# vgteam/vg

Measured on AMD Instinct MI355X. Metric: reads/sec aligned (150 bp), higher is better.
Workload: dtype u16

## Files before the change

include/vgk_engine.h:

```cpp
#ifndef VGK_ENGINE_H
#define VGK_ENGINE_H
#include "vgk.h"
#ifdef __cplusplus
extern "C" {
#endif

typedef struct vgk_find_seeds_policy {
    uint32_t hit_cap, hard_hit_cap;  double minimizer_score_fraction;
    uint32_t max_unique_min, num_bp_per_min, minimizer_coverage_flank, exclude_overlapping_min;
    uint32_t minimizer_downsampling_window_count, reserved;  uint64_t minimizer_downsampling_max_window_length;
} vgk_find_seeds_policy;

#define VGK_SEED_TAKEN        0
#define VGK_SEED_DOWNSAMPLED  1
#define VGK_SEED_NO_HITS      2
#define VGK_SEED_HARD_HIT_CAP 3
#define VGK_SEED_OVERLAPPING  4
#define VGK_SEED_MAX_MIN      5
#define VGK_SEED_HIT_CAP      6

int vgk_minimizer_choose(vgk_ctx* ctx, const vgk_find_seeds_policy* policy, uint32_t k, const char* reads, const uint64_t* read_off, uint32_t n,
                         const uint64_t* minimizer_off, const vgk_read_minimizer* minimizers, uint8_t* verdict);

int vgk_minimizer_find_seeds(vgk_ctx* ctx, const vgk_minimizer_index* index, const vgk_find_seeds_policy* policy, const char* reads, const uint64_t* read_off, uint32_t n,
                             uint64_t* minimizer_off, vgk_read_minimizer* minimizers, uint8_t* take, size_t cap_m,
                             uint64_t* seed_off, vgk_seed* seeds, size_t cap_s, size_t written[2]);

double vgk_minimizer_choose_last_ms(vgk_ctx* ctx);

int vgk_batch_refill_stats(vgk_batch* batch, uint64_t out[5]);

#ifdef __cplusplus
}
#endif
#endif
```

vg_amd/capi.py:

```python
import ctypes
import os
import weakref

import numpy as np

_HERE = os.path.dirname(os.path.abspath(__file__))
DEFAULT_LIB = os.path.join(_HERE, "libvgamd.so")

VGK_OK = 0
VGK_EINVAL, VGK_ENODEV, VGK_ENOMEM, VGK_ETOOLONG, VGK_EOVERFLOW, VGK_EOPS = -1, -2, -3, -4, -5, -6
VGK_GSSW_LOCAL = 0
VGK_GSSW_PINNED = 1
VGK_XDROP_PINNED = 2
VGK_GSSW_TRACEBACK = 16
OP_M, OP_I, OP_D, OP_S = 0, 1, 2, 3
OP_CHARS = "MIDS"

GRAPH_DT = np.dtype([("n_nodes", "<u4"), ("_pad", "<u4"), ("node_len", "<u8"), ("seq", "<u8"),
                     ("pred_off", "<u8"), ("pred_idx", "<u8")])
PROBLEM_DT = np.dtype([("read", "<u8"), ("read_len", "<u4"), ("flags", "<u4"), ("graph", GRAPH_DT), ("pinning", "<u8"),
                       ("max_gap_length", "<u4"), ("reserved", "<u4"), ("qual", "<u8")])
RESULT_DT = np.dtype([("score", "<i4"), ("status", "<i4"), ("end_node", "<i4"), ("end_offset", "<i4"),
                      ("end_read", "<i4"), ("first_offset", "<i4"), ("n_ops", "<u4"), ("ops_begin", "<u4")])
OP_DT = np.dtype([("node", "<u4"), ("len", "<u2"), ("op", "u1"), ("pad", "u1")])
# ... 823 lines not shown
        self.read_off = np.asarray(read_off, dtype=np.int64)
        self.seeds = np.ascontiguousarray(seeds, dtype=SEED_DT)
        self.seed_off = np.asarray(seed_off, dtype=np.int64)
        n = self.n = len(self.read_off) - 1
        arr = np.zeros(n, dtype=GAPLESS_DT)
        arr["read"] = self.reads.ctypes.data + self.read_off[:-1]
        arr["read_len"] = np.diff(self.read_off)
        arr["n_seeds"] = np.diff(self.seed_off)
        arr["seeds"] = self.seeds.ctypes.data + 8 * self.seed_off[:-1]
        arr["max_mismatches"] = max_mismatches
        arr["flags"] = np.where(np.broadcast_to(np.asarray(trim), (n,)), VGK_GAPLESS_TRIM, 0)
        arr["overlap_threshold"] = overlap_threshold
        self.array = arr
        rl = np.diff(self.read_off); ns = np.diff(self.seed_off)
        self.ext_cap = int(ns.sum()) + 1
        self.node_cap = int(node_cap if node_cap is not None else (ns * (rl + 2)).sum()) + 1
        self.mism_cap = int(mism_cap if mism_cap is not None else (ns * rl).sum()) + 1

    @classmethod
    def from_lists(cls, problems):
        reads = [np.frombuffer(p["read"].encode(), dtype=np.uint8) for p in problems]
        read_off = np.concatenate([[0], np.cumsum([len(r) for r in reads])]).astype(np.int64)
        read_buf = np.concatenate(reads) if len(reads) and read_off[-1] else np.zeros(1, np.uint8)
        seed_off = np.concatenate([[0], np.cumsum([len(p["seeds"]) for p in problems])]).astype(np.int64)
        seeds = np.zeros(max(int(seed_off[-1]), 1), dtype=SEED_DT)
        k = 0
        for p in problems:
            for node, diff in p["seeds"]:
                seeds[k] = (node, diff); k += 1
        return cls(read_buf, read_off, seeds, seed_off, [p.get("max_mismatches", 4) for p in problems],
                   [p.get("overlap_threshold", 0.8) for p in problems], [p.get("trim", True) for p in problems])


class WfaSet:

    def __init__(self, seqs, seq_off, mode, from_node, from_offset, to_node, to_offset, path_cap=None, edit_cap=None):
        self.seqs = np.ascontiguousarray(seqs, dtype=np.uint8)
        self.seq_off = np.asarray(seq_off, dtype=np.int64)
        n = self.n = len(self.seq_off) - 1
        arr = np.zeros(n, dtype=WFA_DT)
        arr["seq"] = self.seqs.ctypes.data + self.seq_off[:-1]
        arr["seq_len"] = np.diff(self.seq_off)
        arr["mode"] = mode
        arr["from_node"] = from_node; arr["from_offset"] = from_offset
        arr["to_node"] = to_node; arr["to_offset"] = to_offset
        self.array = arr
        sl = np.diff(self.seq_off)
        self.path_cap = int(path_cap if path_cap is not None else (4 * sl + 64).sum()) + 1
        self.edit_cap = int(edit_cap if edit_cap is not None else (2 * sl + 8).sum()) + 1

    @classmethod
    def from_lists(cls, problems):
        modes = {"connect": WFA_CONNECT, "suffix": WFA_SUFFIX, "prefix": WFA_PREFIX}
        seqs = [np.frombuffer(p["seq"].encode(), dtype=np.uint8) for p in problems]
        seq_off = np.concatenate([[0], np.cumsum([len(r) for r in seqs])]).astype(np.int64)
        buf = np.concatenate(seqs) if len(seqs) and seq_off[-1] else np.zeros(1, np.uint8)
        none = (WFA_NO_NODE, 0)
        return cls(buf, seq_off, [modes[p.get("mode", "connect")] for p in problems],
                   [(p.get("from") or none)[0] for p in problems], [(p.get("from") or none)[1] for p in problems],
                   [(p.get("to") or none)[0] for p in problems], [(p.get("to") or none)[1] for p in problems])


class HaploIndex:

    def __init__(self, eng, nodes, threads=None, gbwt=None):
        self.eng = eng
        if isinstance(nodes, tuple):
            self.nodes = None
            self._len = np.ascontiguousarray(nodes[0], dtype=np.uint32); self._seq = np.ascontiguousarray(nodes[1], dtype=np.uint8)
            nodes = self._len
        else:
            self.nodes = list(nodes)
            self._len = np.array([len(s) for s in nodes], dtype=np.uint32)
            self._seq = np.frombuffer("".join(nodes).encode(), dtype=np.uint8).copy()
        if gbwt is not None:
            h = ctypes.c_void_p()
            eng.lib.vgk_haplo_create_gbwt.argtypes = [ctypes.c_void_p, ctypes.c_char_p, ctypes.c_size_t, ctypes.c_uint32, ctypes.c_void_p, ctypes.c_void_p, ctypes.c_void_p]
            eng._check(eng.lib.vgk_haplo_create_gbwt(eng.h, bytes(gbwt), len(gbwt), len(nodes), self._len.ctypes.data, self._seq.ctypes.data, ctypes.byref(h)),
                       "vgk_haplo_create_gbwt")
            self.h = h
            eng._indexes.add(self)
            return
        self._toff = np.concatenate([[0], np.cumsum([len(t) for t in threads])]).astype(np.uint32)
        self._tn = np.ascontiguousarray(np.concatenate([np.asarray(t, dtype=np.uint32) for t in threads]) if len(threads) and self._toff[-1] else np.zeros(1, np.uint32), dtype=np.uint32)
        d = Haplotypes(len(nodes), self._len.ctypes.data, self._seq.ctypes.data, len(threads), self._toff.ctypes.data, self._tn.ctypes.data)
        h = ctypes.c_void_p()
        eng._check(eng.lib.vgk_haplo_create(eng.h, ctypes.byref(d), ctypes.byref(h)), "vgk_haplo_create")
        self.h = h
        eng._indexes.add(self)

    def run_nodes(self):
        self.eng.lib.vgk_haplo_run_nodes.restype = ctypes.c_uint64; self.eng.lib.vgk_haplo_run_nodes.argtypes = [ctypes.c_void_p]
        return int(self.eng.lib.vgk_haplo_run_nodes(self.h))

    def search_nodes(self):
        self.eng.lib.vgk_haplo_search_nodes.restype = ctypes.c_uint64; self.eng.lib.vgk_haplo_search_nodes.argtypes = [ctypes.c_void_p]
        return int(self.eng.lib.vgk_haplo_search_nodes(self.h))

    def close(self):
        if getattr(self, "h", None):
            if getattr(self.eng, "h", None):
                self.eng.lib.vgk_haplo_destroy(self.h)
            self.h = None

    __del__ = close


class Batch:
    def __init__(self, eng, h, ps, ops_per_problem):
        self.eng, self.h, self.ps, self.ops_per = eng, h, ps, ops_per_problem

    def __enter__(self):
        return self

    def __exit__(self, *a):
        self.free()

    def free(self):
        if self.h:
            self.eng.lib.vgk_batch_free(self.h); self.h = None

    def run(self):
        self.eng._check(self.eng.lib.vgk_gssw_run(self.h), "vgk_gssw_run")

    def sync(self):
        self.eng._check(self.eng.lib.vgk_batch_sync(self.h), "vgk_batch_sync")

    def kernel_ms(self, which=-1):
        return self.eng.lib.vgk_batch_kernel_ms(self.h, which)

    def cells(self):
        return self.eng.lib.vgk_batch_cells(self.h)

    def alg_bytes(self):
        return self.eng.lib.vgk_batch_alg_bytes(self.h)

    def device_bytes(self):
        return self.eng.lib.vgk_batch_device_bytes(self.h)

    def lane(self):
        self.eng.lib.vgk_batch_lane.argtypes = [ctypes.c_void_p]
        return self.eng.lib.vgk_batch_lane(self.h)

    def wave_steps(self):
        return self.eng.lib.vgk_batch_wave_steps(self.h)

    def refill_stats(self):
        f = self.eng.lib.vgk_batch_refill_stats
        f.restype = ctypes.c_int; f.argtypes = [ctypes.c_void_p, ctypes.c_void_p]
        out = (ctypes.c_uint64 * 5)()
        self.eng._check(f(self.h, out), "vgk_batch_refill_stats")
        return dict(zip(("waves", "steps", "missed", "bounded", "broken"), (int(v) for v in out)))

    def speculated(self):
        self.eng.lib.vgk_batch_speculated.argtypes = [ctypes.c_void_p]
        return bool(self.eng.lib.vgk_batch_speculated(self.h))

    def fetch(self, into=None):
        n = self.ps.n
        if self.ops_per:
            cap = n * self.ops_per
        else:
            cap = int(np.diff(self.ps.read_off).sum() + np.diff(self.ps.seq_off).sum() + 2 * n)
        if into is not None:
            res, ops = into[0], (into[1].base if into[1].base is not None else into[1])
            assert len(res) == n and len(ops) >= max(cap, 1)
        else:
            res = np.zeros(n, dtype=RESULT_DT)
            ops = np.zeros(max(cap, 1), dtype=OP_DT)
        written = ctypes.c_size_t()
        self.eng._check(self.eng.lib.vgk_gssw_fetch(self.h, res.ctypes.data, ops.ctypes.data, cap, ctypes.byref(written)),
                        "vgk_gssw_fetch")
        return res, ops[:written.value]


def cigar_string(res_row, ops):
    o = ops[res_row["ops_begin"]:res_row["ops_begin"] + res_row["n_ops"]]
    parts, cur = [], None
    for e in o:
        if cur != e["node"]:
            parts.append("%d:" % e["node"]); cur = e["node"]
        parts[-1] += "%d%s" % (e["len"], OP_CHARS[e["op"]])
    return "%d@%s" % (res_row["first_offset"], ",".join(parts))
```

vg_amd/csrc/backend_hip.hip:

```cpp
#include <chrono>
#include <thread>
#include <hip/hip_runtime.h>
#include <cstdlib>
#include <string>
#include "backend.hpp"
#include "pack_hip.hpp"

namespace vgk {

static __device__ __forceinline__ uint32_t from_lane_above(uint32_t x) {
    return (uint32_t)__builtin_amdgcn_update_dpp(0, (int)x, 0x138 , 0xf, 0xf, true);
}

template <int K>
struct TbStage {
    static constexpr uint32_t REC = (K + 3) / 4, RB = REC - 4;
    static constexpr uint32_t DWORDS = TB_TILE * 64u * REC;
    uint32_t* lds;
    __device__ __forceinline__ uint32_t* slot_a(uint32_t t, uint32_t lane) const { const uint32_t s = t % TB_TILE; return lds + (s * 64u + (lane ^ s)) * 4u; }
    __device__ __forceinline__ uint32_t* slot_b(uint32_t t, uint32_t lane) const { return lds + TB_TILE * 64u * 4u + ((t % TB_TILE) * 64u + lane) * RB; }
    __device__ __forceinline__ void flush(uint32_t* tile, uint32_t lane) const {
        __builtin_amdgcn_fence(__ATOMIC_ACQ_REL, "wavefront");
        __builtin_amdgcn_wave_barrier();
#pragma unroll
        for (uint32_t j = 0; j < TB_TILE; ++j) {
            const uint32_t g = j * 64u + lane, L = g / TB_TILE, s = g % TB_TILE;
            const uint4 v = *reinterpret_cast<const uint4*>(lds + (s * 64u + (L ^ s)) * 4u);
            reinterpret_cast<uint4*>(tile)[g] = v;
        }
        if constexpr (RB > 0) {
            uint32_t* part_b = tile + TB_TILE * 64u * 4u;
            const uint32_t* lb = lds + TB_TILE * 64u * 4u;
#pragma unroll
            for (uint32_t j = 0; j < 2u * RB; ++j) {
                const uint32_t q = j * 64u + lane;
                uint4 v; uint32_t* w = reinterpret_cast<uint32_t*>(&v);
#pragma unroll
                for (uint32_t c = 0; c < 4u; ++c) { const uint32_t d = 4u * q + c, r = d / RB, L = r / TB_TILE, st = r % TB_TILE; w[c] = lb[(st * 64u + L) * RB + d % RB]; }
                reinterpret_cast<uint4*>(part_b)[q] = v;
            }
        }
        __builtin_amdgcn_fence(__ATOMIC_ACQ_REL, "wavefront");
        __builtin_amdgcn_wave_barrier();
    }
};

template <int K, bool S8, bool REWALK, bool CODES = true, bool KEY3 = false, bool NOKEY = false>
__global__ __launch_bounds__(256, (K <= 16 ? 4 : 3)) void gssw_fill_kernel(const GsswParams P) {
    constexpr uint32_t REC = (K + 3) / 4;
    __shared__ __attribute__((aligned(16))) uint32_t stage_lds[4][REWALK ? 64u * TB_BND_CHUNK * 2u : (TB_TILE > 1 ? TbStage<K>::DWORDS : 256u)];
    const uint32_t wave = P.wave_begin + blockIdx.x * 4u + (threadIdx.x >> 6);
    const uint32_t lane = threadIdx.x & 63u;
    if (wave >= P.wave_begin + P.wave_count) return;
    if (P.wave_limit && wave - P.wave_begin >= *P.wave_limit) return;
    const WaveDesc wd = P.waves[wave];
    Lane<K> s;
#if VGK_PB_LDS
    __shared__ uint32_t pb_lds[4][64 * K];
    s.PBL = (typename Lane<K>::lds_u32*)(pb_lds[threadIdx.x >> 6] + lane);
#endif
    lane_init<K, NOKEY ? 1 : 0>(s, P, wd, lane);
    asm volatile("" : "+v"(s.one));
    uint32_t* tb = P.want_tb ? P.tb : nullptr;
    TbStage<K> stage{stage_lds[threadIdx.x >> 6]};
    uint32_t steady_from = 0, steady_to = 0;
    if constexpr (!CODES) {
        uint32_t shortest = s.RA < s.RB ? s.RA : s.RB;
#pragma unroll
        for (int d = 32; d > 0; d >>= 1) { const uint32_t o = (uint32_t)__shfl_xor((int)shortest, d, 64); shortest = o < shortest ? o : shortest; }
        steady_steps(wd.G, shortest, wd.n_steps, steady_from, steady_to);
        steady_from = (uint32_t)__builtin_amdgcn_readfirstlane((int)steady_from); steady_to = (uint32_t)__builtin_amdgcn_readfirstlane((int)steady_to);
    }
    if constexpr (!CODES) {
        uint32_t t = 0;
        for (; t < steady_from; ++t) {
            if ((t & 3u) == 0) lane_prefetch(s, P, t);
            const uint32_t rh = from_lane_above(s.out_h), rf = from_lane_above(s.out_f), ri = from_lane_above(s.info);
            lane_step<K, S8, false, KEY3>(s, P, t, rh, rf, ri, nullptr, nullptr);
        }
        for (; t < steady_to; ++t) {
            if ((t & 3u) == 0) lane_prefetch(s, P, t);
            const uint32_t rh = from_lane_above(s.out_h), rf = from_lane_above(s.out_f), ri = from_lane_above(s.info);
            lane_step<K, S8, false, KEY3, false, true>(s, P, t, rh, rf, ri, nullptr, nullptr);
        }
        for (; t < wd.n_steps; ++t) {
            if ((t & 3u) == 0) lane_prefetch(s, P, t);
            const uint32_t rh = from_lane_above(s.out_h), rf = from_lane_above(s.out_f), ri = from_lane_above(s.info);
            lane_step<K, S8, false, KEY3>(s, P, t, rh, rf, ri, nullptr, nullptr);
        }
    }
    for (uint32_t t = 0; CODES && t < wd.n_steps; ++t) {
        if ((t & 3u) == 0) lane_prefetch(s, P, t);
        const uint32_t rh = from_lane_above(s.out_h);
        const uint32_t rf = from_lane_above(s.out_f);
        const uint32_t ri = from_lane_above(s.info);
        if constexpr (!CODES) {
        } else if constexpr (REWALK) {
            lane_step<K, S8, false>(s, P, t, rh, rf, ri, nullptr, nullptr);
            if (tb) {
                uint32_t* st = stage_lds[threadIdx.x >> 6] + lane * (TB_BND_CHUNK * 2u);
                const uint32_t slot = (t ^ lane) & (TB_BND_CHUNK - 1u);
                *reinterpret_cast<uint2*>(st + slot * 2u) = make_uint2(s.out_h, s.out_f);
                if ((t & (TB_BND_CHUNK - 1u)) == TB_BND_CHUNK - 1u || t + 1u == wd.n_steps) {
                    __builtin_amdgcn_fence(__ATOMIC_ACQ_REL, "wavefront"); __builtin_amdgcn_wave_barrier();
                    uint4* out = reinterpret_cast<uint4*>(tb + tb_bnd(wd.tb_off, wd.n_steps, t & ~(TB_BND_CHUNK - 1u), lane));
#pragma unroll
                    for (uint32_t j = 0; j < TB_BND_CHUNK; j += 2) {
                        const uint2 a = *reinterpret_cast<const uint2*>(st + ((j ^ lane) & (TB_BND_CHUNK - 1u)) * 2u), b = *reinterpret_cast<const uint2*>(st + (((j + 1u) ^ lane) & (TB_BND_CHUNK - 1u)) * 2u);
                        out[j >> 1] = make_uint4(a.x, a.y, b.x, b.y);
                    }
                    __builtin_amdgcn_fence(__ATOMIC_ACQ_REL, "wavefront"); __builtin_amdgcn_wave_barrier();
                }
                lane_store_checkpoint<K>(s, P, wd, t, lane);
            }
        } else if constexpr (TB_TILE > 1) {
            lane_step<K, S8, true, false, NOKEY>(s, P, t, rh, rf, ri, tb ? stage.slot_a(t, lane) : nullptr, stage.slot_b(t, lane));
            if (tb && ((t % TB_TILE) == TB_TILE - 1u || t + 1u == wd.n_steps)) stage.flush(tb + tb_tile_base(wd.tb_off, t, REC), lane);
        } else
            lane_step<K, S8, true, false, NOKEY>(s, P, t, rh, rf, ri, tb ? tb + tb_dword(wd.tb_off, t, lane, REC, 0) : nullptr, tb ? tb + tb_dword(wd.tb_off, t, lane, REC, 4) : nullptr);
    }
    if constexpr (NOKEY) return;
    if (REWALK || !CODES || !P.fused) {
#pragma unroll
        for (int half = 0; half < 2; ++half) {
            uint32_t prob; unsigned long long key;
            if (lane_best(s, half, prob, key)) atomicMax(&P.best[prob], key);
        }
        return;
    }
    unsigned long long* mine = reinterpret_cast<unsigned long long*>(stage_lds[threadIdx.x >> 6]);
#pragma unroll
    for (int half = 0; half < 2; ++half) {
        uint32_t prob; unsigned long long key = 0;
        if (!lane_best(s, half, prob, key)) key = 0;
        mine[lane * 2 + half] = key;
    }
    __threadfence();
    const uint32_t n_slots = 2u * (64u / wd.G);
    for (uint32_t slot = lane; slot < n_slots; slot += 64u) {
        const uint32_t q = slot >> 1, half = slot & 1u;
        if (wd.first_pair + q >= wd.pair_end) continue;
        const uint32_t prob = P.order[2u * (wd.first_pair + q) + half];
        if (prob == 0xffffffffu) continue;
        unsigned long long key = 0;
        for (uint32_t g = 0; g < wd.G; ++g) { const unsigned long long k = mine[(q * wd.G + g) * 2 + half]; key = k > key ? k : key; }
        walk_one(P, prob, key);
    }
}

#ifndef VGK_WALK_WAVES
#define VGK_WALK_WAVES 0
#endif
#if VGK_WALK_WAVES
__global__ __launch_bounds__(256, VGK_WALK_WAVES) void gssw_walk_kernel(const GsswParams P, const int in_fill_order) {
#else
__global__ __launch_bounds__(256) void gssw_walk_kernel(const GsswParams P, const int in_fill_order) {
#endif
    const uint32_t k = blockIdx.x * blockDim.x + threadIdx.x;
    if (!in_fill_order) { if (k < P.n_problems) walk_one(P, k, P.best[k]); return; }
    if (k >= 2u * P.n_pairs) return;
    const uint32_t i = P.order[k];
    if (i != 0xffffffffu) walk_one(P, i, P.best[i]);
}
__global__ __launch_bounds__(64) void banded_geometry_kernel(const BGeomParams P) {
    const uint32_t i = blockIdx.x * blockDim.x + threadIdx.x;
    if (i < P.n) banded_geometry_one(P, i);
}

__global__ __launch_bounds__(64) void gssw_walk_first_kernel(const GsswParams P, const int in_fill_order) {
    __shared__ uint32_t blk[2 * WD_DWORDS * 64];
    __shared__ int16_t tab[WD_TAB];
    if (threadIdx.x < WD_TAB) tab[threadIdx.x] = wd_table_entry(P, threadIdx.x);
    __syncthreads();
    const uint32_t k = blockIdx.x * blockDim.x + threadIdx.x;
    if (!in_fill_order) { if (k < P.n_problems) walk_first_one(P, k, P.best[k], blk + threadIdx.x, 64, tab); return; }
    if (k >= 2u * P.n_pairs) return;
    const uint32_t i = P.order[k];
    if (i != 0xffffffffu) walk_first_one(P, i, P.best[i], blk + threadIdx.x, 64, tab);
}
__global__ __launch_bounds__(64) void gssw_refill_layout_kernel(const GsswParams P) {
    refill_layout_one(P, blockIdx.x * blockDim.x + threadIdx.x);
}
__global__ __launch_bounds__(256) void gssw_refill_restore_kernel(const GsswParams P) {
    const uint32_t i = blockIdx.x * blockDim.x + threadIdx.x;
    if (i < P.n_problems) refill_restore_one(P, i);
}
__global__ __launch_bounds__(256) void gssw_walk_missed_kernel(const GsswParams P) {
    const uint32_t k = blockIdx.x * blockDim.x + threadIdx.x;
    if (k >= *tb_miss_count(P)) return;
    const uint32_t i = tb_miss_list(P)[k];
    walk_one(P, i, P.best[i]);
}

template <int K, bool S8>
__global__ __launch_bounds__(256, 2) void gssw_band_kernel(const GsswParams P) {
    const uint32_t wave = P.wave_begin + blockIdx.x * 4u + (threadIdx.x >> 6);
    if (wave >= P.wave_begin + P.wave_count) return;
    band_fill_lane<K, S8>(P, P.waves[wave], threadIdx.x & 63u);
}
__global__ __launch_bounds__(256) void gssw_bandwalk_kernel(const GsswParams P) {
    const uint32_t k = blockIdx.x * blockDim.x + threadIdx.x;
    if (k >= 2u * P.n_pairs) return;
    const uint32_t i = P.order[k];
    if (i != 0xffffffffu) bandwalk_one(P, i, P.best[i]);
}
template <int K, bool S8>
__global__ __launch_bounds__(64, 2) void gssw_rewalk_kernel(const GsswParams P) {
    __shared__ uint32_t win[(TB_CKPT / 2) * ((K + 3) / 4) * 64];
    const uint32_t count = *tb_miss_count(P);
    const uint32_t* list = tb_miss_list(P);
    for (uint32_t k = blockIdx.x * 64u + threadIdx.x; k < count; k += gridDim.x * 64u) {
        const uint32_t i = list[k];
        rewalk_one<K, S8>(P, i, P.best[i], win + threadIdx.x, 64u);
    }
}

static __device__ __forceinline__ uint32_t ops_of(const vgk_result* res, uint32_t i, uint32_t n) {
    return (i < n && res[i].status == VGK_OK) ? res[i].n_ops : 0u;
}
__global__ __launch_bounds__(256) void ops_scan_kernel(const vgk_result* res, uint32_t n, uint32_t* offs, uint32_t* sums) {
    __shared__ uint32_t wave_total[4];
    const uint32_t i0 = (blockIdx.x * 256u + threadIdx.x) * 4u, lane = threadIdx.x & 63u, w = threadIdx.x >> 6;
    const uint32_t c0 = ops_of(res, i0, n), c1 = ops_of(res, i0 + 1, n), c2 = ops_of(res, i0 + 2, n), c3 = ops_of(res, i0 + 3, n);
    uint32_t incl = c0 + c1 + c2 + c3;
#pragma unroll
    for (uint32_t d = 1; d < 64; d <<= 1) { const uint32_t up = __shfl_up(incl, d, 64); if (lane >= d) incl += up; }
    if (lane == 63) wave_total[w] = incl;
    __syncthreads();
    uint32_t before = 0;
    for (uint32_t k = 0; k < w; ++k) before += wave_total[k];
    uint32_t at = before + incl - (c0 + c1 + c2 + c3);
    if (i0 < n) offs[i0] = at;
    at += c0; if (i0 + 1 < n) offs[i0 + 1] = at;
    at += c1; if (i0 + 2 < n) offs[i0 + 2] = at;
    at += c2; if (i0 + 3 < n) offs[i0 + 3] = at;
    if (threadIdx.x == 255) sums[blockIdx.x] = before + incl;
}
__global__ __launch_bounds__(256) void ops_sums_kernel(uint32_t* sums, uint32_t n_blocks, unsigned long long* total) {
    __shared__ uint32_t wave_total[4];
    __shared__ unsigned long long carry;
    if (threadIdx.x == 0) carry = 0;
    __syncthreads();
    const uint32_t lane = threadIdx.x & 63u, w = threadIdx.x >> 6;
    for (uint32_t base = 0; base < n_blocks; base += 256u) {
        const uint32_t i = base + threadIdx.x;
        const uint32_t c = i < n_blocks ? sums[i] : 0u;
        uint32_t incl = c;
#pragma unroll
        for (uint32_t d = 1; d < 64; d <<= 1) { const uint32_t up = __shfl_up(incl, d, 64); if (lane >= d) incl += up; }
        if (lane == 63) wave_total[w] = incl;
        __syncthreads();
        uint32_t before = 0;
        for (uint32_t k = 0; k < w; ++k) before += wave_total[k];
        const unsigned long long start = carry + before + incl - c;
        if (i < n_blocks) sums[i] = (uint32_t)start;
        __syncthreads();
        if (threadIdx.x == 255) carry += before + incl;
        __syncthreads();
    }
    if (threadIdx.x == 0) *total = carry;
}
__global__ __launch_bounds__(256) void ops_gather_kernel(const vgk_result* res, const vgk_op* ops, uint32_t n, const uint32_t* offs,
                                                         const uint32_t* sums, vgk_result* out_res, vgk_op* out_ops) {
    const uint32_t i = blockIdx.x * blockDim.x + threadIdx.x;
    if (i >= n) return;
    vgk_result r = res[i];
    const uint32_t at = sums[i / Backend::OPS_SCAN_BLOCK] + offs[i];
    if (r.status == VGK_OK && r.n_ops) {
        const vgk_op* from = ops + r.ops_begin;
        for (uint32_t k = 0; k < r.n_ops; ++k) out_ops[at + k] = from[k];
    } else r.n_ops = 0;
    r.ops_begin = at;
// ... 903 lines not shown
    int dev = 0; int n_launches = 1; hipStream_t stream = nullptr, copy = nullptr, fetch = nullptr, side[2] = {nullptr, nullptr}; hipEvent_t side_done[2] = {nullptr, nullptr}; hipEvent_t ev[4] = {nullptr, nullptr, nullptr, nullptr};
    hipStream_t alt = nullptr; hipEvent_t evb[3] = {nullptr, nullptr, nullptr}; float ms_fill_b = 0.f, ms_walk_b = 0.f; bool pending_b = false, timed_walk_b = false, lane1_on_main = true;
    hipEvent_t fill_done[2] = {nullptr, nullptr}; bool fill_done_set[2] = {false, false};
    const bool walk_in_fill_order = std::getenv("VGAMD_WALK_PROBLEM_ORDER") == nullptr;
    const bool fills_take_turns = std::getenv("VGAMD_FILLS_TAKE_TURNS") != nullptr;
    hipDeviceProp_t prop;
    float ms_fill = 0.f, ms_walk = 0.f; bool timed_walk = false, pending = false;
    hipEvent_t sev[2][2] = {{nullptr, nullptr}, {nullptr, nullptr}}; bool sev_set[2] = {false, false}; float ms_refill[2] = {0.f, 0.f};
    float ms_gapless = 0.f, ms_wfa = 0.f, ms_xband = 0.f;
    float ms_bfill = 0.f, ms_bwalk = 0.f; hipEvent_t bev[3] = {nullptr, nullptr, nullptr};
    hipEvent_t xbev[2][2] = {{nullptr, nullptr}, {nullptr, nullptr}};
    hipEvent_t bbev[2][3] = {{nullptr, nullptr, nullptr}, {nullptr, nullptr, nullptr}};
    void* scan_tmp = nullptr; size_t scan_tmp_bytes = 0;
    void* mz_slots = nullptr; size_t mz_slots_bytes = 0;
    void* banded_slab = nullptr; size_t banded_slab_bytes = 0;
    ~HipBackend() override {
        hipSetDevice(dev);
        for (auto& e : ev) if (e) hipEventDestroy(e);
        for (auto& e : bev) if (e) hipEventDestroy(e);
        for (auto& pair : xbev) for (auto& e : pair) if (e) hipEventDestroy(e);
        for (auto& trio : bbev) for (auto& e : trio) if (e) hipEventDestroy(e);
        for (auto& pair : sev) for (auto& e : pair) if (e) hipEventDestroy(e);
        if (scan_tmp) hipFree(scan_tmp);
        if (mz_slots) hipFree(mz_slots);
        if (banded_slab) hipFree(banded_slab);
        for (int i = 0; i < 2; ++i) { if (side[i]) hipStreamDestroy(side[i]); if (side_done[i]) hipEventDestroy(side_done[i]); }
        if (stream) hipStreamDestroy(stream);
        if (copy) hipStreamDestroy(copy);
        if (fetch) hipStreamDestroy(fetch);
        if (alt) hipStreamDestroy(alt);
        for (auto& e : evb) if (e) hipEventDestroy(e);
        for (auto& e : fill_done) if (e) hipEventDestroy(e);
    }
    const char* name() const override { return prop.name; }
    int compute_units() const override { return prop.multiProcessorCount; }
    size_t memory_bytes() const override { return prop.totalGlobalMem; }
    void* alloc(size_t bytes) override {
        hipSetDevice(dev);
        void* p = nullptr;
        if (hipMalloc(&p, bytes ? bytes : 16) != hipSuccess) return nullptr;
        return p;
    }
    void release(void* p) override { if (p) { hipSetDevice(dev); hipFree(p); } }
    void* host_alloc(size_t bytes) override {
        hipSetDevice(dev);
        void* p = nullptr;
        if (hipHostMalloc(&p, bytes ? bytes : 16, hipHostMallocDefault) != hipSuccess) return nullptr;
        return p;
    }
    void host_release(void* p) override { if (p) { hipSetDevice(dev); hipHostFree(p); } }
    int host_register(const void* p, size_t bytes) override { hipSetDevice(dev); return hipHostRegister(const_cast<void*>(p), bytes, hipHostRegisterDefault) == hipSuccess ? VGK_OK : VGK_EINVAL; }
    int host_unregister(const void* p) override { hipSetDevice(dev); return hipHostUnregister(const_cast<void*>(p)) == hipSuccess ? VGK_OK : VGK_EINVAL; }
    int upload(void* dst, const void* src, size_t bytes) override {
        hipSetDevice(dev);
        return hipMemcpyAsync(dst, src, bytes, hipMemcpyHostToDevice, stream) == hipSuccess ? VGK_OK : VGK_ENODEV;
    }
    int upload_side(void* dst, const void* src, size_t bytes) override {
        hipSetDevice(dev);
        return hipMemcpyAsync(dst, src, bytes, hipMemcpyHostToDevice, copy) == hipSuccess ? VGK_OK : VGK_ENODEV;
    }
    void* event_create() override {
        hipSetDevice(dev);
        hipEvent_t e = nullptr;
        return hipEventCreateWithFlags(&e, hipEventDisableTiming) == hipSuccess ? (void*)e : nullptr;
    }
    void event_destroy(void* ev) override { if (ev) { hipSetDevice(dev); hipEventDestroy((hipEvent_t)ev); } }
    int event_record(void* ev) override {
        if (!ev) return VGK_OK;
        hipSetDevice(dev);
        return hipEventRecord((hipEvent_t)ev, stream) == hipSuccess ? VGK_OK : VGK_ENODEV;
    }
    bool event_done(void* ev) override {
        if (!ev) return false;
        hipSetDevice(dev);
        const hipError_t e = hipEventQuery((hipEvent_t)ev);
        if (e != hipSuccess && e != hipErrorNotReady) (void)hipGetLastError();
        return e == hipSuccess;
    }
    int event_wait(void* ev) override {
        if (!ev) return sync();
        hipSetDevice(dev);
        for (;;) {
            const hipError_t e = hipEventQuery((hipEvent_t)ev);
            if (e == hipSuccess) return VGK_OK;
            if (e != hipErrorNotReady) { (void)hipGetLastError(); return VGK_ENODEV; }
            std::this_thread::sleep_for(std::chrono::microseconds(50));
        }
    }
    int fetch_after(void* ev) override {
        if (!ev) return VGK_OK;
        hipSetDevice(dev);
        return hipStreamWaitEvent(fetch, (hipEvent_t)ev, 0) == hipSuccess ? VGK_OK : VGK_ENODEV;
    }
    int sync_fetch() override {
        hipSetDevice(dev);
        return hipStreamSynchronize(fetch) == hipSuccess ? VGK_OK : VGK_ENODEV;
    }
    int download_fetch(void* dst, const void* src, size_t bytes) override {
        hipSetDevice(dev);
        if (hipMemcpyAsync(dst, src, bytes, hipMemcpyDeviceToHost, fetch) != hipSuccess) return VGK_ENODEV;
        return hipStreamSynchronize(fetch) == hipSuccess ? VGK_OK : VGK_ENODEV;
    }
    int download_fetch_async(void* dst, const void* src, size_t bytes) override {
        hipSetDevice(dev);
        return hipMemcpyAsync(dst, src, bytes, hipMemcpyDeviceToHost, fetch) == hipSuccess ? VGK_OK : VGK_ENODEV;
    }
    hipEvent_t side_mark = nullptr;
    int main_after_side() override {
        hipSetDevice(dev);
        if (!side_mark && hipEventCreateWithFlags(&side_mark, hipEventDisableTiming) != hipSuccess) return VGK_ENODEV;
        if (hipEventRecord(side_mark, copy) != hipSuccess || hipStreamWaitEvent(stream, side_mark, 0) != hipSuccess) return VGK_ENODEV;
        return VGK_OK;
    }
    int sync_side() override {
        hipSetDevice(dev);
        return hipStreamSynchronize(copy) == hipSuccess ? VGK_OK : VGK_ENODEV;
    }
    int device_index() const override { return dev; }
    int download(void* dst, const void* src, size_t bytes) override {
        hipSetDevice(dev);
        if (hipMemcpyAsync(dst, src, bytes, hipMemcpyDeviceToHost, stream) != hipSuccess) return VGK_ENODEV;
        return hipStreamSynchronize(stream) == hipSuccess ? VGK_OK : VGK_ENODEV;
    }
    int zero(void* dst, size_t bytes) override {
        hipSetDevice(dev);
        if (bytes >= ((size_t)1 << 18) && ((uintptr_t)dst & 15u) == 0) {
            const size_t vecs = bytes / 16;
            const unsigned blocks = (unsigned)std::min<size_t>((vecs + 255) / 256, (size_t)std::max(1, prop.multiProcessorCount) * 8);
            hipLaunchKernelGGL(zero_kernel, dim3(blocks), dim3(256), 0, stream, (uint4*)dst, vecs, (unsigned char*)dst + vecs * 16, (uint32_t)(bytes - vecs * 16));
            return hipGetLastError() == hipSuccess ? VGK_OK : VGK_ENODEV;
        }
        return hipMemsetAsync(dst, 0, bytes, stream) == hipSuccess ? VGK_OK : VGK_ENODEV;
    }
    int sync() override {
        hipSetDevice(dev);
        return hipStreamSynchronize(stream) == hipSuccess ? VGK_OK : VGK_ENODEV;
    }
    size_t win_tmp_bytes(uint32_t n, uint32_t n_waves_cap) override { hipSetDevice(dev); return hip_win_tmp_bytes(n, n_waves_cap); }
    int win_stage1(const WinParams& P, void* tmp, size_t tmp_bytes) override { hipSetDevice(dev); return hip_win_stage1(P, tmp, tmp_bytes, copy); }
    int win_stage2(const WinParams& P, void* tmp, size_t tmp_bytes) override { hipSetDevice(dev); return hip_win_stage2(P, tmp, tmp_bytes, copy); }
    int download_side(void* dst, const void* src, size_t bytes) override {
        hipSetDevice(dev);
        if (hipMemcpyAsync(dst, src, bytes, hipMemcpyDeviceToHost, copy) != hipSuccess) return VGK_ENODEV;
        return hipStreamSynchronize(copy) == hipSuccess ? VGK_OK : VGK_ENODEV;
    }
    int fill_side(void* dst, int byte, size_t bytes) override {
        hipSetDevice(dev);
        return hipMemsetAsync(dst, byte, bytes, copy) == hipSuccess ? VGK_OK : VGK_ENODEV;
    }
    template <int K> int launch_fill_k(const GsswParams& p, hipStream_t stream) {
        const dim3 grid((p.wave_count + 3) / 4), block(256);
        const bool s8 = p.scale == 8, re = p.tb_mode == TB_REWALK;
        if (p.spec_fill == 1) {
            if (s8 && p.key3) hipLaunchKernelGGL((gssw_fill_kernel<K, true, false, false, true>), grid, block, 0, stream, p);
            else if (s8) hipLaunchKernelGGL((gssw_fill_kernel<K, true, false, false>), grid, block, 0, stream, p); else hipLaunchKernelGGL((gssw_fill_kernel<K, false, false, false>), grid, block, 0, stream, p);
            return VGK_OK;
        }
        if (p.spec_fill == 2 && s8 && !re && !p.fused) { hipLaunchKernelGGL((gssw_fill_kernel<K, true, false, true, false, true>), grid, block, 0, stream, p); return VGK_OK; }
        if (re) { if (s8) hipLaunchKernelGGL((gssw_fill_kernel<K, true, true>), grid, block, 0, stream, p); else hipLaunchKernelGGL((gssw_fill_kernel<K, false, true>), grid, block, 0, stream, p); }
        else    { if (s8) hipLaunchKernelGGL((gssw_fill_kernel<K, true, false>), grid, block, 0, stream, p); else hipLaunchKernelGGL((gssw_fill_kernel<K, false, false>), grid, block, 0, stream, p); }
        return VGK_OK;
    }
    int launch_fill(const GsswParams& p, hipStream_t stream) {
        switch (p.K) {
            case 16: return launch_fill_k<16>(p, stream);
            case 19: return launch_fill_k<19>(p, stream);
            case 20: return launch_fill_k<20>(p, stream);
            case 24: return launch_fill_k<24>(p, stream);
            default: return VGK_EINVAL;
        }
    }
    template <int K> void launch_rewalk_k(const GsswParams& p, hipStream_t stream) {
        const dim3 grid(1024), block(64);
        if (p.scale == 8) hipLaunchKernelGGL((gssw_rewalk_kernel<K, true>), grid, block, 0, stream, p); else hipLaunchKernelGGL((gssw_rewalk_kernel<K, false>), grid, block, 0, stream, p);
    }
    template <int K> void launch_band_k(const GsswParams& p, hipStream_t stream) {
        const dim3 grid((p.wave_count + 3) / 4), block(256);
        if (p.scale == 8) hipLaunchKernelGGL((gssw_band_kernel<K, true>), grid, block, 0, stream, p); else hipLaunchKernelGGL((gssw_band_kernel<K, false>), grid, block, 0, stream, p);
    }
    void launch_walk(const GsswParams& p0, const FillLaunch* launches, uint32_t n, hipStream_t stream, int lane = 0) {
        sev_set[lane] = false;
        if (p0.tb_mode != TB_REWALK) {
            if (p0.walk_passes == 2) {
                hipLaunchKernelGGL(gssw_walk_first_kernel, dim3((2 * p0.n_pairs + 63) / 64), dim3(64), 0, stream, p0, walk_in_fill_order ? 1 : 0);
                if (p0.spec_fill) {
                    const uint32_t max_waves = (p0.n_pairs + 64u / p0.refill_G - 1u) / (64u / p0.refill_G);
                    for (int k = 0; k < 2; ++k) if (!sev[lane][k]) hipEventCreate(&sev[lane][k]);
                    hipEventRecord(sev[lane][0], stream);
                    hipLaunchKernelGGL(gssw_refill_layout_kernel, dim3((max_waves + 63) / 64), dim3(64), 0, stream, p0);
                    GsswParams p = p0;
                    p.spec_fill = 2; p.K = p0.refill_K; p.wave_begin = p0.refill_wave0; p.wave_count = max_waves; p.wave_limit = p0.refill_count;
                    launch_fill(p, stream);
                    hipEventRecord(sev[lane][1], stream); sev_set[lane] = true;
                }
                hipLaunchKernelGGL(gssw_walk_missed_kernel, dim3((p0.n_problems + 255) / 256), dim3(256), 0, stream, p0);
            } else hipLaunchKernelGGL(gssw_walk_kernel, dim3((2 * p0.n_pairs + 255) / 256), dim3(256), 0, stream, p0, walk_in_fill_order ? 1 : 0);
            return;
        }
        GsswParams p = p0;
        for (uint32_t i = 0; i < n; ++i) {
            if (!launches[i].wave_count) continue;
            p.K = launches[i].K; p.wave_begin = launches[i].wave_begin; p.wave_count = launches[i].wave_count;
            switch (p.K) { case 16: launch_band_k<16>(p, stream); break; case 19: launch_band_k<19>(p, stream); break; case 20: launch_band_k<20>(p, stream); break; case 24: launch_band_k<24>(p, stream); break; default: break; }
        }
        hipLaunchKernelGGL(gssw_bandwalk_kernel, dim3((2 * p0.n_pairs + 255) / 256), dim3(256), 0, stream, p0);
        for (uint32_t i = 0; i < n; ++i) {
            if (!launches[i].wave_count) continue;
            p.K = launches[i].K; p.wave_begin = launches[i].wave_begin; p.wave_count = launches[i].wave_count;
            switch (p.K) { case 16: launch_rewalk_k<16>(p, stream); break; case 19: launch_rewalk_k<19>(p, stream); break; case 20: launch_rewalk_k<20>(p, stream); break; case 24: launch_rewalk_k<24>(p, stream); break; default: break; }
        }
    }
    int run_gssw(const GsswParams& p0, const FillLaunch* launches, uint32_t n, bool walk) override {
        hipSetDevice(dev);
        n_launches = n ? (int)n : 1;
        if (p0.n_problems == 0 || n == 0) { ms_fill = ms_walk = 0; pending = false; return VGK_OK; }
        GsswParams p = p0;
        if (p0.restore_probs) hipLaunchKernelGGL(gssw_refill_restore_kernel, dim3((p0.n_problems + 255) / 256), dim3(256), 0, stream, p0);
        if (fills_take_turns && fill_done_set[1]) hipStreamWaitEvent(stream, fill_done[1], 0);
        hipEventRecord(ev[0], stream);
        for (uint32_t i = 0; i < n; ++i) {
            const FillLaunch& L = launches[i];
            p.K = L.K; p.wave_begin = L.wave_begin; p.wave_count = L.wave_count;
            if (L.wave_count == 0) continue;
            hipStream_t st = (i == 0 || i > 2) ? stream : side[i - 1];
            if (st != stream) hipStreamWaitEvent(st, ev[0], 0);
            int rc = launch_fill(p, st);
            if (rc) return rc;
            if (st != stream) { hipEventRecord(side_done[i - 1], st); hipStreamWaitEvent(stream, side_done[i - 1], 0); }
        }
        hipEventRecord(ev[1], stream);
        hipEventRecord(fill_done[0], stream); fill_done_set[0] = true;
        timed_walk = walk && (!p.fused || p.tb_mode == TB_REWALK);
        if (timed_walk) {
            launch_walk(p0, launches, n, stream);
            hipEventRecord(ev[2], stream);
        }
        pending = true;
        return hipGetLastError() == hipSuccess ? VGK_OK : VGK_ENODEV;
    }
    int run_gssw_on(int lane, const GsswParams& p0, const FillLaunch* launches, uint32_t n, bool walk, void* done) override {
        hipSetDevice(dev);
        if (lane != 1 || n != 1 || p0.n_problems == 0) {
            if (lane == 1) lane1_on_main = true;
            if (hipMemsetAsync(p0.best, 0, ((size_t)p0.n_problems + 1) * sizeof(unsigned long long), stream) != hipSuccess) return VGK_ENODEV;
            int rc = run_gssw(p0, launches, n, walk);
            if (!rc && done) rc = hipEventRecord((hipEvent_t)done, stream) == hipSuccess ? VGK_OK : VGK_ENODEV;
            return rc;
        }
        lane1_on_main = false;
        if (hipMemsetAsync(p0.best, 0, ((size_t)p0.n_problems + 1) * sizeof(unsigned long long), alt) != hipSuccess) return VGK_ENODEV;
        GsswParams p = p0;
        p.K = launches[0].K; p.wave_begin = launches[0].wave_begin; p.wave_count = launches[0].wave_count;
        if (p0.restore_probs) hipLaunchKernelGGL(gssw_refill_restore_kernel, dim3((p0.n_problems + 255) / 256), dim3(256), 0, alt, p0);
        if (fills_take_turns && fill_done_set[0]) hipStreamWaitEvent(alt, fill_done[0], 0);
        hipEventRecord(evb[0], alt);
        if (p.wave_count) { const int rc = launch_fill(p, alt); if (rc) return rc; }
        hipEventRecord(evb[1], alt);
        hipEventRecord(fill_done[1], alt); fill_done_set[1] = true;
        timed_walk_b = walk && (!p.fused || p.tb_mode == TB_REWALK);
        if (timed_walk_b) {
            launch_walk(p0, launches, n, alt, 1);
            hipEventRecord(evb[2], alt);
        }
        pending_b = true;
        if (done && hipEventRecord((hipEvent_t)done, alt) != hipSuccess) return VGK_ENODEV;
        return hipGetLastError() == hipSuccess ? VGK_OK : VGK_ENODEV;
    }
    double last_ms_on(int lane, int which) const override {
        if (which == 12) {
            const int l = (lane == 1 && !lane1_on_main) ? 1 : 0;
            HipBackend* self = const_cast<HipBackend*>(this);
            if (!sev_set[l]) return 0.0;
            hipSetDevice(dev); hipStreamSynchronize(l ? alt : stream);
            float ms = 0.f; if (hipEventElapsedTime(&ms, sev[l][0], sev[l][1]) != hipSuccess) { (void)hipGetLastError(); ms = 0.f; }
            self->ms_refill[l] = ms; return ms;
        }
        if (lane != 1 || lane1_on_main || which > 2 || which < 0) return last_ms(which);
        HipBackend* self = const_cast<HipBackend*>(this);
        if (self->pending_b) {
            hipSetDevice(dev);
            hipStreamSynchronize(alt);
            hipEventElapsedTime(&self->ms_fill_b, evb[0], evb[1]);
            self->ms_walk_b = 0.f;
            if (timed_walk_b) hipEventElapsedTime(&self->ms_walk_b, evb[1], evb[2]);
            self->pending_b = false;
        }
        return which == 0 ? ms_fill_b : which == 1 ? ms_walk_b : 1.0;
    }
    int ops_offsets(const vgk_result* res, uint32_t n, uint32_t* offs, uint32_t* sums, uint64_t* total) override {
        hipSetDevice(dev);
        const uint32_t blocks = (n + OPS_SCAN_BLOCK - 1) / OPS_SCAN_BLOCK;
        unsigned long long* total_dev = (unsigned long long*)(sums + ((blocks + 2) & ~1u));
        hipLaunchKernelGGL(ops_scan_kernel, dim3(blocks), dim3(256), 0, fetch, res, n, offs, sums);
        hipLaunchKernelGGL(ops_sums_kernel, dim3(1), dim3(256), 0, fetch, sums, blocks, total_dev);
        unsigned long long t = 0;
        if (hipMemcpyAsync(&t, total_dev, sizeof t, hipMemcpyDeviceToHost, fetch) != hipSuccess) return VGK_ENODEV;
        if (hipStreamSynchronize(fetch) != hipSuccess || hipGetLastError() != hipSuccess) return VGK_ENODEV;
        *total = t;
        return VGK_OK;
    }
    int ops_gather(const vgk_result* res, const vgk_op* ops, uint32_t n, const uint32_t* offs, const uint32_t* sums, vgk_result* out_res, vgk_op* out_ops) override {
        hipSetDevice(dev);
        hipLaunchKernelGGL(ops_gather_kernel, dim3((n + 255) / 256), dim3(256), 0, fetch, res, ops, n, offs, sums, out_res, out_ops);
        return hipGetLastError() == hipSuccess ? VGK_OK : VGK_ENODEV;
    }
    int run_banded(const BandedParams& p, const BandedLaunch* launches, uint32_t n) override {
        ms_bfill = ms_bwalk = 0.f;
// ... 374 lines not shown
```

vg_amd/csrc/gssw_device.hpp:

```cpp
#pragma once
#include <stdint.h>
#include "../../include/vgk.h"
#include "pk16.hpp"

namespace vgk {

constexpr int KMAX = 24;

constexpr uint32_t XOFF = 1023;

enum : uint32_t {
    CI_BASE_MASK  = 7,
    CI_NODE_START = 8,
    CI_STORE_END  = 16,
    CI_SEED_SLOW  = 32,
    CI_INVALID    = 128
};
constexpr uint32_t CI_INVALID2 = CI_INVALID | (CI_INVALID << 16);

struct ProbDesc {
    uint32_t col_off;
    uint32_t R;
    uint32_t L;
    uint32_t read_off;
    uint32_t node_off;
    uint32_t n_nodes;
    uint32_t scratch_off;
    uint32_t n_slots;
    uint32_t flags;
    uint32_t ops_off;
    uint32_t ops_cap;
    uint32_t max_gap;
    uint32_t wave;
    uint32_t lane0;
    uint32_t geom;
    uint32_t Lpad;
    uint32_t bonus_start, bonus_end;
    uint32_t prof_off;
    uint32_t pad;
    uint32_t col0, node0;
};

struct NodeRec {
    uint32_t col_start;
    uint32_t col_end;
    uint32_t pred_begin;
    uint32_t n_pred;
    int32_t  slot;
    uint32_t pinning;
};

struct WaveDesc {
    uint64_t tb_off;
    uint32_t n_steps;
    uint32_t first_pair;
    uint32_t G;
    uint32_t pair_end;
};

struct GsswParams {
    const ProbDesc* probs;
    const uint8_t*  colinfo;
    const uint8_t*  reads;
    const uint32_t* prof;
    const NodeRec*  nodes;
    const uint32_t* preds;
    uint32_t*       scratch;
    uint32_t*       tb;
    const WaveDesc* waves;
    const uint32_t* order;
    unsigned long long* best;
    vgk_result*     results;
    vgk_op*         ops;
    uint32_t n_problems, n_pairs, n_waves;
    uint32_t wave_begin, wave_count;
    uint32_t K;
    uint32_t prof4[6];
    uint32_t bias;
    uint32_t go, ge;
    int32_t  bonus;
    int32_t  want_tb;
    int32_t  spec_fill;
    uint32_t key3;
    int32_t  restore_probs;
    uint32_t refill_wave0, refill_pair0, refill_G, refill_K;
    unsigned long long refill_slot;
    uint32_t* refill_count;
    int32_t  refill_bound;
    uint32_t refill_m;
    const uint32_t* wave_limit;
    int32_t  walk_passes;
    int32_t  tb_mode;
    int32_t  dbg;
    int32_t  fused;
    uint32_t scale;
    uint32_t xoff;
    int8_t   matrix[25];
};

VGK_HD uint32_t rep2(uint32_t x) { return (x & 0xffffu) * 0x00010001u; }

struct ProfWords {
    uint32_t w0, w1, w2, w3, w4;
    VGK_HD uint32_t of(uint32_t q) const {
        uint32_t a = w0, b = w1, c = w2, e = w3, f = w4;
#if defined(__HIP_DEVICE_COMPILE__)
        asm volatile("" : "+v"(a), "+v"(b), "+v"(c), "+v"(e), "+v"(f));
#endif
        uint32_t w = a; w = q == 1 ? b : w; w = q == 2 ? c : w; w = q == 3 ? e : w; w = q == 4 ? f : w;
        return w;
    }
    VGK_HD uint32_t of_row(uint32_t q) const { return q == 5 ? 0u : of(q); }
};
VGK_HD ProfWords prof_words(const GsswParams& P) { return ProfWords{P.prof4[0], P.prof4[1], P.prof4[2], P.prof4[3], P.prof4[4]}; }

VGK_HD uint32_t row_bonus(uint32_t bonus_start, uint32_t bonus_end, uint32_t row, uint32_t L) {
    return (row == 0 ? bonus_start : 0u) + (row + 1 == L ? bonus_end : 0u);
}

VGK_HD unsigned long long key64(uint32_t score, uint32_t col, uint32_t row) {
    return ((unsigned long long)score << 40) | ((unsigned long long)(0xFFFFFu - col) << 20) | (unsigned long long)(0xFFFFFu - row);
}

#ifndef VGK_PB_LDS
#define VGK_PB_LDS 0
#endif
template <int K>
struct Lane {
    uint32_t H[K];
    uint32_t E[K];
    uint32_t PA[K];
#if VGK_PB_LDS && defined(__HIPCC__)
    typedef __attribute__((address_space(3))) uint32_t lds_u32;
    lds_u32* PBL;
    VGK_HD uint32_t pb(int m) const { return *(const volatile lds_u32*)(PBL + 64 * m); }
    VGK_HD void set_pb(int m, uint32_t v) { PBL[64 * m] = v; }
#else
    uint32_t PB[K];
    VGK_HD uint32_t pb(int m) const { return PB[m]; }
    VGK_HD void set_pb(int m, uint32_t v) { PB[m] = v; }
#endif
    uint32_t out_h, out_f, info;
    uint32_t prev_rh;
    uint32_t best_lo, best_hi, step_lo, step_hi;
    uint32_t nodeA, nodeB;
    uint32_t g;
    uint32_t Lpad;
    uint32_t probA, probB;
    uint32_t LA, LB, flagsA, flagsB;
    uint32_t bsA, beA, bsB, beB;
    uint32_t RA, RB, colA, colB;
    uint32_t ciA, ciB, ciA_n, ciB_n;
    uint32_t one;
};

VGK_HD uint32_t ci_word(uint32_t w, uint32_t t, uint32_t R) {
    const uint32_t none = CI_INVALID * 0x01010101u;
    if (t + 4u <= R) return w;
    if (t >= R) return none;
    const uint32_t keep = (1u << (8u * (R - t))) - 1u;
    return (w & keep) | (none & ~keep);
}
template <int K, int SECOND = -1>
VGK_HD void lane_init(Lane<K>& s, const GsswParams& P, const WaveDesc& wd, uint32_t lane_id) {
    const uint32_t q = lane_id / wd.G;
    s.g = lane_id - q * wd.G;
    s.Lpad = wd.G * K;
    const uint32_t pair = wd.first_pair + q;
    const bool live = (q < 64u / wd.G) && (pair < wd.pair_end);
    s.probA = live ? P.order[2 * pair] : 0xffffffffu;
    s.probB = live ? P.order[2 * pair + 1] : 0xffffffffu;
    s.LA = s.LB = 0; s.flagsA = s.flagsB = 0; s.RA = s.RB = 0; s.colA = s.colB = 0;
    s.ciA = s.ciB = s.ciA_n = s.ciB_n = CI_INVALID * 0x01010101u;
    uint32_t roA = 0, roB = 0, poA = 0xffffffffu, poB = 0xffffffffu;
    uint32_t c0A = 0, c0B = 0, n0A = 0, n0B = 0;
    s.bsA = s.beA = s.bsB = s.beB = 0;
    if (s.probA != 0xffffffffu) { const ProbDesc& d = P.probs[s.probA]; s.LA = d.L; s.flagsA = d.flags; roA = d.read_off; s.RA = d.R; s.colA = d.col_off;
                                   s.bsA = d.bonus_start; s.beA = d.bonus_end; poA = d.prof_off; if (SECOND > 0 || (SECOND < 0 && P.spec_fill == 2)) { c0A = d.col0; n0A = d.node0; } }
    if (s.probB != 0xffffffffu) { const ProbDesc& d = P.probs[s.probB]; s.LB = d.L; s.flagsB = d.flags; roB = d.read_off; s.RB = d.R; s.colB = d.col_off;
                                   s.bsB = d.bonus_start; s.beB = d.bonus_end; poB = d.prof_off; if (SECOND > 0 || (SECOND < 0 && P.spec_fill == 2)) { c0B = d.col0; n0B = d.node0; } }
    if (SECOND != 0) {
        s.colA += c0A; s.RA -= c0A; s.colB += c0B; s.RB -= c0B;
        if (c0A) s.flagsA = VGK_GSSW_PINNED;
        if (c0B) s.flagsB = VGK_GSSW_PINNED;
    }
    if (s.g == 0) {
        if (s.probA != 0xffffffffu) s.ciA_n = ci_word(*(const uint32_t*)(P.colinfo + s.colA), 0, s.RA);
        if (s.probB != 0xffffffffu) s.ciB_n = ci_word(*(const uint32_t*)(P.colinfo + s.colB), 0, s.RB);
    }
    const ProfWords pw = prof_words(P);
#pragma unroll
    for (int m = 0; m < K; ++m) {
        const uint32_t row = s.g * K + m;
        uint32_t pa = 0, pb = 0;
        if (row < s.LA) pa = poA != 0xffffffffu ? P.prof[poA + row] : pw.of_row(P.reads[roA + row]) + 0x01010101u * row_bonus(s.bsA, s.beA, row, s.LA);
        if (row < s.LB) pb = poB != 0xffffffffu ? P.prof[poB + row] : pw.of_row(P.reads[roB + row]) + 0x01010101u * row_bonus(s.bsB, s.beB, row, s.LB);
        s.PA[m] = pa; s.set_pb(m, pb); s.H[m] = 0; s.E[m] = 0;
    }
    s.out_h = 0; s.out_f = 0; s.info = CI_INVALID2; s.prev_rh = 0;
    s.best_lo = s.best_hi = 0; s.step_lo = s.step_hi = 0;
    s.nodeA = SECOND != 0 ? n0A - 1u : 0xffffffffu; s.nodeB = SECOND != 0 ? n0B - 1u : 0xffffffffu;
    s.one = 0x00010001u;
}

template <int K>
VGK_HD void lane_prefetch(Lane<K>& s, const GsswParams& P, uint32_t t) {
    if (s.g != 0) return;
    s.ciA = s.ciA_n; s.ciB = s.ciB_n;
    s.ciA_n = t + 4 < s.RA ? ci_word(*(const uint32_t*)(P.colinfo + s.colA + t + 4), t + 4, s.RA) : CI_INVALID * 0x01010101u;
    s.ciB_n = t + 4 < s.RB ? ci_word(*(const uint32_t*)(P.colinfo + s.colB + t + 4), t + 4, s.RB) : CI_INVALID * 0x01010101u;
}

template <int K>
VGK_HD uint32_t fetch_info(const Lane<K>& s, const GsswParams& P, uint32_t t) {
    (void)P;
    return byte_perm(s.ciB, s.ciA, 0x0c040c00u + (t & 3u) * 0x00010001u);
}

#if defined(__HIP_DEVICE_COMPILE__)
static __device__ __forceinline__ uint32_t scratch_load(const uint32_t* p) {
    return __hip_atomic_load(p, __ATOMIC_RELAXED, __HIP_MEMORY_SCOPE_AGENT);
}
#else
static inline uint32_t scratch_load(const uint32_t* p) { return *p; }
#endif

template <int HALF, int K>
VGK_HD void seed_from_scratch(Lane<K>& s, const GsswParams& P, uint32_t prob, uint32_t node, uint32_t& diag0) {
    const ProbDesc& d = P.probs[prob];
    const NodeRec& nr = P.nodes[d.node_off + node];
    const uint32_t keep = HALF == 0 ? 0xffff0000u : 0x0000ffffu;
#pragma unroll
    for (int m = 0; m < K; ++m) { s.H[m] &= keep; s.E[m] &= keep; }
    diag0 &= keep;
    if (nr.n_pred == 0 && (d.flags & 15u) == VGK_XDROP_PINNED) {
#pragma unroll
        for (int m = 0; m <= K; ++m) {
            const uint32_t row = s.g * K + m - 1;
            uint32_t h = 0;
            if (m > 0 || s.g > 0) {
                if (row == 0) h = P.xoff;
                else if (row <= d.max_gap) { const uint32_t pen = P.go + (row - 1) * P.ge; h = pen < P.xoff ? P.xoff - pen : 0; }
            }
            if (m == 0) { diag0 |= HALF == 0 ? h : (h << 16); }
            else {
                const uint32_t e = h > P.go ? h - P.go : 0;
                s.H[m - 1] |= HALF == 0 ? h : (h << 16);
                s.E[m - 1] |= HALF == 0 ? e : (e << 16);
            }
        }
        return;
    }
    for (uint32_t k = 0; k < nr.n_pred; ++k) {
        const NodeRec& pr = P.nodes[d.node_off + P.preds[nr.pred_begin + k]];
        const uint32_t* base = P.scratch + d.scratch_off + (uint32_t)pr.slot * s.Lpad + s.g * K;
#pragma unroll
        for (int m = 0; m < K; ++m) {
            const uint32_t v = scratch_load(base + m);
            s.H[m] = pk_max(s.H[m], HALF == 0 ? (v & 0xffffu) : (v << 16));
            s.E[m] = pk_max(s.E[m], HALF == 0 ? (v >> 16) : (v & 0xffff0000u));
        }
        if (s.g > 0) {
            const uint32_t v = scratch_load(base - 1);
            diag0 = pk_max(diag0, HALF == 0 ? (v & 0xffffu) : (v << 16));
        }
    }
}

template <int HALF, int K>
VGK_HD void store_to_scratch(const Lane<K>& s, const GsswParams& P, uint32_t prob, uint32_t node) {
    const ProbDesc& d = P.probs[prob];
    const NodeRec& nr = P.nodes[d.node_off + node];
    uint32_t* base = P.scratch + d.scratch_off + (uint32_t)nr.slot * s.Lpad + s.g * K;
#pragma unroll
    for (int m = 0; m < K; ++m) {
        uint32_t h = HALF == 0 ? (s.H[m] & 0xffffu) : (s.H[m] >> 16);
        uint32_t e = HALF == 0 ? (s.E[m] & 0xffffu) : (s.E[m] >> 16);
        base[m] = h | (e << 16);
    }
}

#ifndef VGK_TB_TILED
#define VGK_TB_TILED 0
#endif
struct alignas(16) VgkU4 { uint32_t v[4]; };
constexpr uint32_t TB_TILE = VGK_TB_TILED ? 8 : 1;
VGK_HD uint64_t tb_tile_base(uint64_t tb_off, uint32_t t, uint32_t rec_dwords) { return tb_off + (uint64_t)(t / TB_TILE) * (64u * TB_TILE * rec_dwords); }
VGK_HD uint64_t tb_dword(uint64_t tb_off, uint32_t t, uint32_t lane, uint32_t rec_dwords, uint32_t j) {
    if (TB_TILE == 1) return tb_off + ((uint64_t)t * 64u + lane) * rec_dwords + j;
    const uint64_t base = tb_tile_base(tb_off, t, rec_dwords);
    const uint32_t at = lane * TB_TILE + t % TB_TILE;
    return j < 4u ? base + at * 4u + j : base + 64u * TB_TILE * 4u + at * (rec_dwords - 4u) + (j - 4u);
}

#ifndef VGK_ACC_SHLOR
#define VGK_ACC_SHLOR 0
#endif
#ifndef VGK_H_MAX3
#define VGK_H_MAX3 1
#endif

VGK_HD bool gssw_key3_ok(uint32_t scale, bool quality_adjusted, bool any_xdrop, uint32_t longest_read, uint32_t max_score, uint32_t max_bonus) {
    return scale == 8u && !quality_adjusted && !any_xdrop && (uint64_t)longest_read * max_score + 2ull * max_bonus <= 990ull;
}
constexpr uint32_t KEY_SHIFT = 5, KEY_LOW = 31;

template <int K, int M, bool REFN, bool S8, bool TB>
VGK_HD uint32_t row_diag(const Lane<K>& s, const GsswParams& P, uint32_t sel, uint32_t bias2, bool nA, bool nB, uint32_t d) {
    uint32_t sb = byte_perm(s.pb(M), s.PA[M], sel);
    if (REFN) {
        const uint32_t row = s.g * K + M;
        if (nA) sb = set_lo(sb, row < s.LA ? P.bias + row_bonus(s.bsA, s.beA, row, s.LA) : 0u);
        if (nB) sb = set_hi(sb, row < s.LB ? P.bias + row_bonus(s.bsB, s.beB, row, s.LB) : 0u);
    }
    return pk_subs(pk_add_nc(d, sb), (TB && S8) ? bias2 - 0x00040004u : bias2);
}
template <int K, int M, bool REFN, bool S8, bool TB, bool K3, bool NK>
VGK_HD void lane_row(Lane<K>& s, const GsswParams& P, uint32_t sel, uint32_t bias2, uint32_t go2, uint32_t ge2,
                     bool nA, bool nB, uint32_t& f, uint32_t& d, uint32_t* acc, uint32_t& ck) {
    const uint32_t t4 = d;
    if constexpr (M + 1 < K) d = row_diag<K, M + 1, REFN, S8, TB>(s, P, sel, bias2, nA, nB, s.H[M]);
    if constexpr (!TB) {
        const uint32_t e = s.E[M];
        const uint32_t h = (S8 && VGK_H_MAX3) ? pk_max3_f16(t4, e, f) : pk_max(pk_max(t4, e), f);
        const uint32_t gg = pk_subs(h, go2);
        const uint32_t en = pk_max(gg, pk_subs(e, ge2)), fn = pk_max(gg, pk_subs(f, ge2));
        const uint32_t key = pk_mad_add_imm<(int)KEY_LOW - M>(h, 0x00010001u << (S8 ? KEY_SHIFT - 3 : KEY_SHIFT));
        if constexpr (S8 && K3) {
            if constexpr ((M & 1) == 0) { if constexpr (M + 1 < K) acc[0] = key; else ck = M == 0 ? key : pk_max(ck, key); }
            else ck = M == 1 ? pk_max(acc[0], key) : pk_max3_f16(ck, acc[0], key);
        } else ck = M == 0 ? key : pk_max(ck, key);
        s.H[M] = h; s.E[M] = en; f = fn;
        return;
    }
    if constexpr (S8) {
        const uint32_t ei = s.E[M] | 0x00030003u;
        const uint32_t h = VGK_H_MAX3 ? pk_max3_f16(t4, ei, f) : pk_max(pk_max(t4, ei), f);
        const uint32_t hc = h & 0xfff8fff8u;
        const uint32_t gg = pk_subs(hc, go2 - 0x00010001u);
        const uint32_t e2 = pk_subs(ei, ge2 + 0x00030003u), f2 = pk_subs(f | 0x00010001u, ge2 + 0x00010001u);
        const uint32_t en = pk_max(gg, e2), fn = pk_max(gg, f2);
        uint32_t code = bit_select<0x00010001u>(en, h) & 0x00070007u;
        code = shl_or<3>(fn & 0x00010001u, code);
        acc[M >> 2] = (M & 3) == 0 ? code : (VGK_ACC_SHLOR ? shl_or<4>(acc[M >> 2], code) : pk_mul_add_imm<16>(acc[M >> 2], code));
        if constexpr (!NK) {
            const uint32_t key = pk_mad_add_imm<(int)KEY_LOW - M>(hc, 0x00010001u << (KEY_SHIFT - 3));
            ck = M == 0 ? key : pk_max(ck, key);
        }
        s.H[M] = hc; s.E[M] = en; f = fn;
        return;
    }
    const uint32_t e = s.E[M];
    const uint32_t h = pk_max(pk_max(t4, e), f);
    const uint32_t gg = pk_subs(h, go2);
    const uint32_t e2 = pk_subs(e, ge2), f2 = pk_subs(f, ge2);
    const uint32_t en = pk_max(gg, e2), fn = pk_max(gg, f2);
    const uint32_t one = s.one;
    const uint32_t nd = pk_min(pk_sub_nb(h, t4), one);
    const uint32_t ne = pk_min(pk_sub_nb(h, e), one);
    const uint32_t eb = pk_min(pk_sub_nb(en, gg), one);
    const uint32_t fb = pk_min(pk_sub_nb(fn, gg), one);
    uint32_t code = pk_mul_add_imm<2>(ne, nd); code = pk_mul_add_imm<4>(eb, code); code = pk_mul_add_imm<8>(fb, code);
    acc[M >> 2] = (M & 3) == 0 ? code : pk_mul_add_imm<16>(acc[M >> 2], code);
    const uint32_t key = pk_mad_add_imm<(int)KEY_LOW - M>(h, 0x00010001u << KEY_SHIFT);
    ck = M == 0 ? key : pk_max(ck, key);
    s.H[M] = h; s.E[M] = en; f = fn;
}

template <int K, int M, bool REFN, bool S8, bool TB, bool K3, bool NK>
VGK_HD void lane_rows_from(Lane<K>& s, const GsswParams& P, uint32_t sel, uint32_t bias2, uint32_t go2, uint32_t ge2,
                           bool nA, bool nB, uint32_t& f, uint32_t& d, uint32_t* acc, uint32_t& ck) {
    lane_row<K, M, REFN, S8, TB, K3, NK>(s, P, sel, bias2, go2, ge2, nA, nB, f, d, acc, ck);
    if constexpr (M + 1 < K) lane_rows_from<K, M + 1, REFN, S8, TB, K3, NK>(s, P, sel, bias2, go2, ge2, nA, nB, f, d, acc, ck);
}

template <int K, bool REFN, bool S8, bool TB, bool K3, bool NK>
VGK_HD void lane_rows(Lane<K>& s, const GsswParams& P, uint32_t sel, uint32_t diag0, uint32_t rf,
                      bool nA, bool nB, uint32_t* acc, uint32_t& colkey) {
    uint32_t bias2 = rep2(P.bias), go2 = rep2(P.go), ge2 = rep2(P.ge);
#if defined(__HIP_DEVICE_COMPILE__)
    if (REFN) asm volatile("" : "+v"(sel), "+v"(bias2), "+v"(go2), "+v"(ge2));
#endif
    uint32_t f = rf, d = row_diag<K, 0, REFN, S8, TB>(s, P, sel, bias2, nA, nB, diag0), ck = 0;
    lane_rows_from<K, 0, REFN, S8, TB, K3, NK>(s, P, sel, bias2, go2, ge2, nA, nB, f, d, acc, ck);
    s.out_h = s.H[K - 1]; s.out_f = f;
    colkey = ck;
}

template <int K, bool S8, bool TB, bool RE, bool K3 = false, bool NK = false, bool AV = false>
VGK_HD void lane_column(Lane<K>& s, const GsswParams& P, uint32_t t, uint32_t rh, uint32_t rf, uint32_t rinfo, uint32_t* tb_a, uint32_t* tb_b) {
    s.info = rinfo;
    const uint32_t ia = rinfo & 0xffu, ib = (rinfo >> 16) & 0xffu;
    const bool vA = AV || !(ia & CI_INVALID), vB = AV || !(ib & CI_INVALID);
    if (AV || vA || vB) {
        uint32_t diag0 = s.prev_rh;
        if (vA && (ia & CI_NODE_START)) s.nodeA += 1;
        if (vB && (ib & CI_NODE_START)) s.nodeB += 1;
        if (rinfo & (CI_SEED_SLOW * 0x00010001u)) {
            if (vA && (ia & CI_SEED_SLOW)) seed_from_scratch<0, K>(s, P, s.probA, s.nodeA, diag0);
            if (vB && (ib & CI_SEED_SLOW)) seed_from_scratch<1, K>(s, P, s.probB, s.nodeB, diag0);
        }
        const uint32_t sel = (rinfo & 0x00030003u) | 0x0c040c00u;
        uint32_t acc[(K + 3) / 4], colkey;
        if (rinfo & 0x00040004u) { const bool nA = (ia & CI_BASE_MASK) == 4, nB = (ib & CI_BASE_MASK) == 4; lane_rows<K, true, S8, TB, K3, NK>(s, P, sel, diag0, rf, nA, nB, acc, colkey); }
        else          lane_rows<K, false, S8, TB, K3, NK>(s, P, sel, diag0, rf, false, false, acc, colkey);
        if constexpr (TB) {
            if (tb_a) {
                if (TB_TILE > 1 && !RE) {
                    VgkU4 v; v.v[0] = acc[0]; v.v[1] = acc[1]; v.v[2] = acc[2]; v.v[3] = acc[3];
                    *reinterpret_cast<VgkU4*>(tb_a) = v;
#pragma unroll
                    for (int j = 4; j < (K + 3) / 4; ++j) tb_b[j - 4] = acc[j];
                } else {
#pragma unroll
                    for (int j = 0; j < (K + 3) / 4; ++j) { if (j < 4) tb_a[j] = acc[j]; else tb_b[j - 4] = acc[j]; }
                }
            }
        }
        if constexpr (!RE) {
            if constexpr (!NK) {
            const uint32_t klo = colkey & 0xffffu, khi = colkey >> 16;
            const bool upA = vA & ((klo >> KEY_SHIFT) > (s.best_lo >> KEY_SHIFT)), upB = vB & ((khi >> KEY_SHIFT) > (s.best_hi >> KEY_SHIFT));
            s.best_lo = upA ? klo : s.best_lo; s.step_lo = upA ? t : s.step_lo;
            s.best_hi = upB ? khi : s.best_hi; s.step_hi = upB ? t : s.step_hi;
            }
            if (rinfo & (CI_STORE_END * 0x00010001u)) {
                if (vA && (ia & CI_STORE_END)) store_to_scratch<0, K>(s, P, s.probA, s.nodeA);
                if (vB && (ib & CI_STORE_END)) store_to_scratch<1, K>(s, P, s.probB, s.nodeB);
            }
        }
    } else {
        s.out_h = 0; s.out_f = 0;
    }
    s.prev_rh = rh;
}

VGK_HD void steady_steps(uint32_t G, uint32_t shortest, uint32_t n_steps, uint32_t& from, uint32_t& to) {
    from = G - 1u < n_steps ? G - 1u : n_steps; to = shortest < n_steps ? shortest : n_steps; if (to < from) to = from;
}
template <int K, bool S8, bool TB = true, bool K3 = false, bool NK = false, bool AV = false>
VGK_HD void lane_step(Lane<K>& s, const GsswParams& P, uint32_t t, uint32_t rh, uint32_t rf, uint32_t rinfo, uint32_t* tb_a, uint32_t* tb_b) {
    if (s.g == 0) { rh = 0; rf = 0; rinfo = fetch_info(s, P, t); }
    lane_column<K, S8, TB, false, K3, NK, AV>(s, P, t, rh, rf, rinfo, tb_a, tb_b);
}

template <int K>
VGK_HD bool lane_best(const Lane<K>& s, int half, uint32_t& prob, unsigned long long& key) {
    const uint32_t b = half ? s.best_hi : s.best_lo, st = half ? s.step_hi : s.step_lo;
    prob = half ? s.probB : s.probA;
    if (prob == 0xffffffffu || (b >> KEY_SHIFT) == 0) return false;
    const uint32_t L = half ? s.LB : s.LA, flags = half ? s.flagsB : s.flagsA;
    if ((flags & 15u) == VGK_GSSW_PINNED) return false;
    const uint32_t row = s.g * K + (KEY_LOW - (b & KEY_LOW));
    if (row >= L) return false;
    key = key64(b >> KEY_SHIFT, st - s.g, row);
    return true;
}

#ifndef VGK_WALK_SPEC
#define VGK_WALK_SPEC 8
#endif
constexpr uint32_t W_SPEC = VGK_WALK_SPEC;
constexpr uint32_t W_MISS = 0x100u;
struct Walker {
    static constexpr uint32_t SPEC = W_SPEC;
    const GsswParams& P; const ProbDesc& d; uint32_t half, lane0, K; uint64_t tb_off;
    VGK_HD uint32_t code(uint32_t r, uint32_t c) const {
        if (c < d.col0) return W_MISS;
        const uint32_t g = r / K, m = r - g * K, t = c - d.col0 + g, j = m >> 2, i = m & 3u;
#if defined(VGK_WALK_EXP) && VGK_WALK_EXP >= 1
        const uint32_t w = P.tb[tb_off + (tb_dword(0, t, lane0 + g, (K + 3) >> 2, j) & (VGK_WALK_EXP == 1 ? 0x3ffffu : 0xfffu))];
#else
#if defined(__HIP_DEVICE_COMPILE__) && !defined(VGK_WALK_PLAIN_LOADS)
        const uint32_t w = __builtin_nontemporal_load(&P.tb[tb_dword(tb_off, t, lane0 + g, (K + 3) >> 2, j)]);
#else
        const uint32_t w = P.tb[tb_dword(tb_off, t, lane0 + g, (K + 3) >> 2, j)];
#endif
#endif
        const uint32_t last = (4 * j + 3 < K ? 4 * j + 3 : K - 1) - 4 * j;
        const uint32_t raw = (w >> (16 * half + 4 * (last - i))) & 15u;
        if (P.scale != 8) return raw;
        const uint32_t src = (raw >> 1) & 3u;
        return (src != 2u ? 1u : 0u) | (src == 0u ? 2u : 0u) | ((raw & 1u) ? 0u : 4u) | ((raw & 8u) ? 0u : 8u);
    }
    mutable uint32_t rd_word = 0, rd_base = 0xffffffffu, ci_word = 0, ci_base = 0xffffffffu;
    const ProfWords pw = prof_words(P);
    VGK_HD uint32_t read_code(uint32_t r) const {
        const uint32_t a = d.read_off + r, b = a & ~3u;
        if (b != rd_base) { rd_base = b; rd_word = *(const uint32_t*)(P.reads + b); }
        return (rd_word >> (8 * (a & 3u))) & 0xffu;
    }
    VGK_HD uint32_t col_base(uint32_t c) const {
        const uint32_t a = d.col_off + c, b = a & ~3u;
        if (b != ci_base) { ci_base = b; ci_word = *(const uint32_t*)(P.colinfo + b); }
        return (ci_word >> (8 * (a & 3u))) & CI_BASE_MASK;
    }
    VGK_HD int32_t score(uint32_t r, uint32_t c) const {
#if defined(VGK_WALK_EXP) && VGK_WALK_EXP == 3
        return (int32_t)((r ^ c) & 1u) * 5 - 4;
#endif
        const uint32_t base = col_base(c);
        const int32_t bonus = (int32_t)row_bonus(d.bonus_start, d.bonus_end, r, d.L);
        if (base >= 4) return bonus;
        if (d.prof_off != 0xffffffffu)
            return (int32_t)((P.prof[d.prof_off + r] >> (8 * base)) & 0xffu) - (int32_t)P.bias;
        const uint32_t q = read_code(r);
        return (int32_t)((pw.of(q) >> (8 * base)) & 0xffu) - (int32_t)P.bias + bonus;
    }
    VGK_HD uint32_t saved(const NodeRec& n, uint32_t r) const { return P.scratch[d.scratch_off + (uint32_t)n.slot * d.Lpad + r]; }
    VGK_HD int32_t saved_e(const NodeRec& n, uint32_t r) const {
        const uint32_t v = saved(n, r) >> 16;
        return (int32_t)(P.scale == 8 ? v & ~7u : v);
    }
};

template <class SAVED>
VGK_HD bool walk_end_cell(const GsswParams& P, const ProbDesc& d, unsigned long long best_key, SAVED saved, int32_t& cur, uint32_t& c, uint32_t& node, int32_t& r) {
    const NodeRec* nodes = P.nodes + d.node_off;
    bool have = false;
    cur = 0; c = 0; node = 0; r = 0;
    if ((d.flags & 15u) == VGK_GSSW_PINNED) {
        r = (int32_t)d.L - 1;
        for (uint32_t n = 0; n < d.n_nodes; ++n) {
            if (!nodes[n].pinning) continue;
            const int32_t v = (int32_t)(saved(nodes[n], (uint32_t)r) & 0xffffu);
            if (!have || v > cur) { cur = v; node = n; have = true; }
        }
        if (have) c = nodes[node].col_end - 1;
    } else {
        const unsigned long long k = best_key;
        cur = (int32_t)(k >> 40) * (int32_t)P.scale;
        if (cur > 0) {
            have = true;
            c = 0xFFFFFu - (uint32_t)((k >> 20) & 0xFFFFFu);
            r = (int32_t)(0xFFFFFu - (uint32_t)(k & 0xFFFFFu));
            uint32_t lo = 0, hi = d.n_nodes;
            while (hi - lo > 1) { const uint32_t mid = (lo + hi) >> 1; if (nodes[mid].col_start <= c) lo = mid; else hi = mid; }
            node = lo;
        }
    }
    return have;
}

constexpr int32_t  W_MISSED = 100;

template <class W>
VGK_HD int32_t walk_body(const GsswParams& P, uint32_t i, const ProbDesc& d, W& w, unsigned long long best_key) {
    constexpr uint32_t W_SPEC = W::SPEC;
    vgk_result res;
    res.score = 0; res.status = VGK_OK; res.end_node = -1; res.end_offset = -1; res.end_read = -1;
    res.first_offset = 0; res.n_ops = 0; res.ops_begin = d.ops_off;
    const NodeRec* nodes = P.nodes + d.node_off;
    const bool pinned = (d.flags & 15u) == VGK_GSSW_PINNED;
    const bool xdrop = (d.flags & 15u) == VGK_XDROP_PINNED;
    const int32_t go = (int32_t)P.go, ge = (int32_t)P.ge;
    const int32_t S = (int32_t)P.scale;
    const int32_t zero = xdrop ? (int32_t)P.xoff : 0;

    int32_t cur = 0; uint32_t c = 0, node = 0; int32_t r = 0;
    const bool have = walk_end_cell(P, d, best_key, [&](const NodeRec& n, uint32_t row) { return w.saved(n, row); }, cur, c, node, r);
    if (pinned && !have) { res.status = VGK_EINVAL; P.results[i] = res; return VGK_EINVAL; }
    if (cur >= 2047 * S) { res.status = VGK_EOVERFLOW; P.results[i] = res; return VGK_EOVERFLOW; }
    if (!have || cur <= zero) { P.results[i] = res; return VGK_OK; }
    res.score = (cur - zero) / S; res.end_node = (int32_t)node; res.end_offset = (int32_t)(c - nodes[node].col_start);
    res.end_read = xdrop ? r - 1 : r;
    if (!(d.flags & VGK_GSSW_TRACEBACK)) { P.results[i] = res; return VGK_OK; }

    vgk_op* ops = P.ops + d.ops_off;
    uint32_t pos = d.ops_cap;
    int32_t status = VGK_OK;
    uint32_t rn = 0, ro = 0xffu, rl = 0;
#define VGK_FLUSH() do { if (rl) { if (pos == 0) status = VGK_EOPS; else { --pos; \
        ops[pos].node = rn; ops[pos].len = (uint16_t)rl; ops[pos].op = (uint8_t)ro; ops[pos].pad = 0; } } } while (0)
#define VGK_PUSH(NODE, OP, LEN) do { \
        if (rl && rn == (uint32_t)(NODE) && ro == (uint32_t)(OP)) rl += (LEN); \
        else { VGK_FLUSH(); rn = (uint32_t)(NODE); ro = (uint32_t)(OP); rl = (LEN); } } while (0)

    if (r < (int32_t)d.L - 1) VGK_PUSH(node, VGK_OP_S, d.L - 1 - (uint32_t)r);
    enum { ST_H, ST_E, ST_F } st = ST_H;
    bool at_root = false;
    uint32_t first_c = c;
    uint32_t node_start = nodes[node].col_start;
    for (uint32_t guard = 0; guard < 2 * (d.L + d.R) + 4 && status == VGK_OK; ++guard) {
        const bool first = (c == node_start);
        (void)first;
        if (st == ST_H) {
            if (!xdrop && cur == 0) break;
            const uint32_t room = c - node_start + 1, rows = (uint32_t)r + 1;
            uint32_t nspec = room < rows ? room : rows; nspec = nspec < W_SPEC ? nspec : W_SPEC;
            uint32_t fl[W_SPEC]; int32_t sc[W_SPEC];
#pragma unroll
            for (uint32_t k = 0; k < W_SPEC; ++k) {
                fl[k] = 1u; sc[k] = 0;
                if (k < nspec) { fl[k] = w.code((uint32_t)r - k, c - k); sc[k] = w.score((uint32_t)r - k, c - k); }
            }
#if defined(VGK_DEBUG_WALK) && !defined(__HIP_DEVICE_COMPILE__)
// ... 186 lines not shown
    if (!b.used) return b;
    const uint32_t r_hi = g * K + K - 1u < r_e ? g * K + K - 1u : r_e;
    const uint32_t back_lo = r_e - g * K + TB_SLACK, back_hi = r_e - r_hi;
    const uint32_t lo = c_e > back_lo ? c_e - back_lo : 0u;
    uint32_t hi = c_e > back_hi ? c_e - back_hi + TB_SLACK : TB_SLACK;
    if (hi > c_e) hi = c_e;
    b.cs = lo / TB_CKPT * TB_CKPT;
    const uint32_t last = b.cs + tb_band_cols(K) - 1u;
    b.hi = hi < last ? hi : last;
    return b;
}

constexpr uint32_t TB_BND_CHUNK = 16;
VGK_HD uint32_t tb_steps_padded(uint32_t n_steps) { return (n_steps + TB_BND_CHUNK - 1u) / TB_BND_CHUNK * TB_BND_CHUNK; }
VGK_HD uint64_t tb_bnd_dwords(uint32_t n_steps) { return 128ull * tb_steps_padded(n_steps); }

VGK_HD uint64_t tb_wave_dwords(uint32_t n_steps, uint32_t K) {
    const uint64_t rec = (K + 3u) >> 2;
    const uint64_t codes = (uint64_t)((n_steps + TB_TILE - 1) / TB_TILE * TB_TILE) * 64u * rec;
    const uint64_t rewalk = tb_bnd_dwords(n_steps) + (uint64_t)((n_steps + TB_CKPT - 1) / TB_CKPT) * 128u * K + 64ull * tb_band_cols(K) * rec;
    return codes > rewalk ? codes : rewalk;
}
VGK_HD uint64_t tb_bnd(uint64_t tb_off, uint32_t n_steps, uint32_t t, uint32_t lane) { return tb_off + ((uint64_t)lane * tb_steps_padded(n_steps) + t) * 2u; }
VGK_HD uint64_t tb_ckpt(uint64_t tb_off, uint32_t n_steps, uint32_t cb, uint32_t lane, uint32_t K) {
    return tb_off + tb_bnd_dwords(n_steps) + ((uint64_t)cb * 64u + lane) * 2u * K;
}
VGK_HD uint64_t tb_band(uint64_t tb_off, uint32_t n_steps, uint32_t x, uint32_t lane, uint32_t K) {
    return tb_off + tb_bnd_dwords(n_steps) + (uint64_t)((n_steps + TB_CKPT - 1) / TB_CKPT) * 128u * K + ((uint64_t)x * 64u + lane) * ((K + 3u) >> 2);
}

template <int K>
VGK_HD void lane_store_boundary(const Lane<K>& s, const GsswParams& P, const WaveDesc& wd, uint32_t t, uint32_t lane) {
    uint32_t* b = P.tb + tb_bnd(wd.tb_off, wd.n_steps, t, lane);
    b[0] = s.out_h; b[1] = s.out_f;
}
template <int K>
VGK_HD void lane_store_checkpoint(const Lane<K>& s, const GsswParams& P, const WaveDesc& wd, uint32_t t, uint32_t lane) {
    const uint32_t c = t - s.g;
    if (t >= s.g && (c & (TB_CKPT - 1u)) == TB_CKPT - 1u && !((s.info & CI_INVALID) && (s.info & (CI_INVALID << 16)))) {
        uint32_t* k = P.tb + tb_ckpt(wd.tb_off, wd.n_steps, c / TB_CKPT, lane, (uint32_t)K);
#pragma unroll
        for (int m = 0; m < K; ++m) { k[m] = s.H[m]; k[K + m] = s.E[m]; }
    }
}

template <int K, bool S8>
struct ReWalker {
    static constexpr uint32_t SPEC = 1;
    static constexpr uint32_t REC = (K + 3) / 4;
    Walker base;
    uint32_t* win; uint32_t win_stride;
    uint32_t n_steps;
    uint32_t win_g = 0xffffffffu, win_c0 = 0, win_hi = 0;
    Lane<K> ln;

    VGK_HD int32_t score(uint32_t r, uint32_t c) const { return base.score(r, c); }
    VGK_HD uint32_t saved(const NodeRec& n, uint32_t r) const { return base.saved(n, r); }
    VGK_HD int32_t saved_e(const NodeRec& n, uint32_t r) const { return base.saved_e(n, r); }

    VGK_HD uint32_t code(uint32_t r, uint32_t c) {
        const uint32_t g = r / K, m = r - g * K, j = m >> 2, i = m & 3u;
        if (g != win_g || c < win_c0 || c > win_hi) refill(g, c);
        const uint32_t x = c - win_c0;
        const uint32_t w = (win[((x >> 1) * REC + j) * win_stride] >> (16u * (x & 1u))) & 0xffffu;
        const uint32_t last = (4 * j + 3 < (uint32_t)K ? 4 * j + 3 : (uint32_t)K - 1) - 4 * j;
        const uint32_t raw = (w >> (4 * (last - i))) & 15u;
        if (!S8) return raw;
        const uint32_t src = (raw >> 1) & 3u;
        return (src != 2u ? 1u : 0u) | (src == 0u ? 2u : 0u) | ((raw & 1u) ? 0u : 4u) | ((raw & 8u) ? 0u : 8u);
    }

    VGK_HD void refill(uint32_t g, uint32_t c) {
        const GsswParams& P = base.P; const ProbDesc& d = base.d;
        const uint32_t half = base.half, lane = base.lane0 + g;
        const uint64_t tb_off = base.tb_off;
#if VGK_PB_LDS && defined(__HIPCC__)
        ln.PBL = (typename Lane<K>::lds_u32*)(uintptr_t)0;
#endif
        const uint32_t c0 = c / TB_CKPT * TB_CKPT;
        Lane<K>& s = ln;
        s.g = g; s.Lpad = d.Lpad;
        s.probA = half ? 0xffffffffu : 0u; s.probB = half ? 0u : 0xffffffffu;
        s.LA = s.LB = 0; s.flagsA = s.flagsB = 0; s.RA = s.RB = 0; s.colA = s.colB = 0; s.ciA = s.ciB = s.ciA_n = s.ciB_n = 0;
        s.bsA = s.beA = s.bsB = s.beB = 0;
        if (half) { s.probB = prob_index; s.LB = d.L; s.flagsB = d.flags; s.RB = d.R; s.colB = d.col_off; s.bsB = d.bonus_start; s.beB = d.bonus_end; }
        else      { s.probA = prob_index; s.LA = d.L; s.flagsA = d.flags; s.RA = d.R; s.colA = d.col_off; s.bsA = d.bonus_start; s.beA = d.bonus_end; }
        const uint32_t keep = half ? 0xffff0000u : 0x0000ffffu;
        const uint32_t* ck = c0 ? P.tb + tb_ckpt(tb_off, n_steps, c0 / TB_CKPT - 1u, lane, (uint32_t)K) : nullptr;
#pragma unroll
        for (int m = 0; m < K; ++m) {
            const uint32_t row = g * K + m;
            uint32_t pw = 0;
            if (row < d.L) pw = d.prof_off != 0xffffffffu ? P.prof[d.prof_off + row] : P.prof4[P.reads[d.read_off + row]] + 0x01010101u * row_bonus(d.bonus_start, d.bonus_end, row, d.L);
            s.PA[m] = half ? 0u : pw; s.set_pb(m, half ? pw : 0u);
            s.H[m] = ck ? ck[m] & keep : 0u; s.E[m] = ck ? ck[K + m] & keep : 0u;
        }
        s.out_h = 0; s.out_f = 0; s.info = CI_INVALID2;
        s.best_lo = s.best_hi = 0; s.step_lo = s.step_hi = 0;
        s.one = 0x00010001u;
#if defined(__HIP_DEVICE_COMPILE__)
        asm volatile("" : "+v"(s.one));
#endif
        uint32_t node = 0xffffffffu;
        if (c0) {
            const NodeRec* nodes = P.nodes + d.node_off;
            uint32_t lo = 0, hi = d.n_nodes;
            while (hi - lo > 1) { const uint32_t mid = (lo + hi) >> 1; if (nodes[mid].col_start <= c0 - 1u) lo = mid; else hi = mid; }
            node = lo;
        }
        s.nodeA = s.nodeB = node;
        s.prev_rh = (c0 && g) ? P.tb[tb_bnd(tb_off, n_steps, c0 - 1u + g - 1u, lane - 1u)] & keep : 0u;
        uint32_t pend[REC];
        for (uint32_t col = c0; col <= c; ++col) {
            const uint32_t t = col + g;
            uint32_t rh = 0, rf = 0;
            if (g) { const uint32_t* b = P.tb + tb_bnd(tb_off, n_steps, t - 1u, lane - 1u); rh = b[0] & keep; rf = b[1] & keep; }
            const uint32_t ci = P.colinfo[d.col_off + col];
            const uint32_t rinfo = half ? ((uint32_t)CI_INVALID | (ci << 16)) : (ci | ((uint32_t)CI_INVALID << 16));
            uint32_t rec[REC];
            lane_column<K, S8, true, true>(s, P, t, rh, rf, rinfo, rec, rec + 4);
            const uint32_t x = col - c0;
#pragma unroll
            for (uint32_t j = 0; j < REC; ++j) {
                const uint32_t v = (rec[j] >> (16u * half)) & 0xffffu;
                if (x & 1u) win[((x >> 1) * REC + j) * win_stride] = pend[j] | (v << 16);
                else pend[j] = v;
            }
        }
        if (!((c - c0) & 1u)) {
#pragma unroll
            for (uint32_t j = 0; j < REC; ++j) win[(((c - c0) >> 1) * REC + j) * win_stride] = pend[j];
        }
        win_g = g; win_c0 = c0; win_hi = c;
    }
    uint32_t prob_index = 0;
};

VGK_HD bool tb_band_end(const GsswParams& P, const ProbDesc& d, unsigned long long best_key, uint32_t& r_e, uint32_t& c_e) {
    if (!(d.flags & VGK_GSSW_TRACEBACK)) return false;
    int32_t cur, r; uint32_t c, node;
    const bool have = walk_end_cell(P, d, best_key, [&](const NodeRec& n, uint32_t row) { return P.scratch[d.scratch_off + (uint32_t)n.slot * d.Lpad + row]; }, cur, c, node, r);
    const int32_t zero = (d.flags & 15u) == VGK_XDROP_PINNED ? (int32_t)P.xoff : 0;
    if (!have || cur <= zero || cur >= 2047 * (int32_t)P.scale || r < 0) return false;
    r_e = (uint32_t)r; c_e = c;
    return true;
}

template <int K, bool S8>
VGK_HD void band_fill_lane(const GsswParams& P, const WaveDesc& wd, uint32_t lane) {
    Lane<K> s;
#if VGK_PB_LDS && defined(__HIPCC__)
    s.PBL = (typename Lane<K>::lds_u32*)(uintptr_t)0;
#endif
    lane_init(s, P, wd, lane);
    const uint32_t g = s.g;
    uint32_t re[2] = {0, 0}, ce[2] = {0, 0}; TbBand bd[2]; bd[0].used = bd[1].used = false;
    const uint32_t prob[2] = {s.probA, s.probB};
#pragma unroll
    for (int h = 0; h < 2; ++h) {
        if (prob[h] == 0xffffffffu) continue;
        const ProbDesc& d = P.probs[prob[h]];
        if (tb_band_end(P, d, P.best[prob[h]], re[h], ce[h])) bd[h] = tb_band_of(re[h], ce[h], g, (uint32_t)K);
    }
    if (!bd[0].used && !bd[1].used) return;
    uint32_t prev = 0;
#pragma unroll
    for (int h = 0; h < 2; ++h) {
        const uint32_t keep = h ? 0xffff0000u : 0x0000ffffu;
        uint32_t node = 0xffffffffu;
        if (bd[h].used && bd[h].cs) {
            const ProbDesc& d = P.probs[prob[h]];
            const uint32_t* ck = P.tb + tb_ckpt(wd.tb_off, wd.n_steps, bd[h].cs / TB_CKPT - 1u, lane, (uint32_t)K);
#pragma unroll
            for (int m = 0; m < K; ++m) { s.H[m] |= ck[m] & keep; s.E[m] |= ck[K + m] & keep; }
            const NodeRec* nodes = P.nodes + d.node_off;
            uint32_t lo = 0, hi = d.n_nodes;
            while (hi - lo > 1) { const uint32_t mid = (lo + hi) >> 1; if (nodes[mid].col_start <= bd[h].cs - 1u) lo = mid; else hi = mid; }
            node = lo;
            if (g) prev |= P.tb[tb_bnd(wd.tb_off, wd.n_steps, bd[h].cs - 1u + g - 1u, lane - 1u)] & keep;
        }
        if (h) s.nodeB = node; else s.nodeA = node;
    }
    s.prev_rh = prev;
    uint32_t n_col[2]; const uint8_t* ci_at[2]; const uint32_t* up_at[2];
#pragma unroll
    for (int h = 0; h < 2; ++h) {
        n_col[h] = bd[h].used ? bd[h].hi - bd[h].cs + 1u : 0u;
        ci_at[h] = nullptr; up_at[h] = nullptr;
        if (n_col[h]) {
            ci_at[h] = P.colinfo + P.probs[prob[h]].col_off + bd[h].cs;
            if (g) up_at[h] = P.tb + tb_bnd(wd.tb_off, wd.n_steps, bd[h].cs + g - 1u, lane - 1u);
        }
    }
    uint32_t n_max = n_col[0] > n_col[1] ? n_col[0] : n_col[1];
    if ((P.dbg & 1) && n_max > 1u) n_max = 1u;
    struct In { uint32_t rinfo, rh, rf; };
    auto fetch = [&](uint32_t x) {
        In in; in.rinfo = CI_INVALID2; in.rh = 0; in.rf = 0;
#pragma unroll
        for (int h = 0; h < 2; ++h) {
            if (x >= n_col[h]) continue;
            const uint32_t ci = ci_at[h][x];
            in.rinfo = h ? (in.rinfo & 0x0000ffffu) | (ci << 16) : (in.rinfo & 0xffff0000u) | ci;
            if (up_at[h]) {
                const uint32_t keep = h ? 0xffff0000u : 0x0000ffffu;
                in.rh |= up_at[h][2u * x] & keep; in.rf |= up_at[h][2u * x + 1u] & keep;
            }
        }
        return in;
    };
    uint32_t* out = P.tb + tb_band(wd.tb_off, wd.n_steps, 0, lane, (uint32_t)K);
    constexpr uint32_t OUT_STRIDE = 64u * ((K + 3) / 4);
    In next = fetch(0);
    for (uint32_t x = 0; x < n_max; ++x, out += OUT_STRIDE) {
        const In in = next;
        if (x + 1u < n_max) next = fetch(x + 1u);
        lane_column<K, S8, true, true>(s, P, x, in.rh, in.rf, in.rinfo, (P.dbg & 2) ? nullptr : out, out + 4);
    }
}

struct BandWalker {
    static constexpr uint32_t SPEC = W_SPEC;
    Walker base;
    uint32_t n_steps, r_e, c_e;
    mutable uint32_t bg = 0xffffffffu; mutable TbBand bb{0, 0, false};
    VGK_HD int32_t score(uint32_t r, uint32_t c) const { return base.score(r, c); }
    VGK_HD uint32_t saved(const NodeRec& n, uint32_t r) const { return base.saved(n, r); }
    VGK_HD int32_t saved_e(const NodeRec& n, uint32_t r) const { return base.saved_e(n, r); }
    VGK_HD uint32_t code(uint32_t r, uint32_t c) const {
        const uint32_t K = base.K, g = r / K, m = r - g * K, j = m >> 2, i = m & 3u;
        if (g != bg) { bg = g; bb = tb_band_of(r_e, c_e, g, K); }
        if (!bb.used || c < bb.cs || c > bb.hi) return W_MISS;
        const uint32_t w = base.P.tb[tb_band(base.tb_off, n_steps, c - bb.cs, base.lane0 + g, K) + j];
        const uint32_t last = (4 * j + 3 < K ? 4 * j + 3 : K - 1) - 4 * j;
        const uint32_t raw = (w >> (16 * base.half + 4 * (last - i))) & 15u;
        if (base.P.scale != 8) return raw;
        const uint32_t src = (raw >> 1) & 3u;
        return (src != 2u ? 1u : 0u) | (src == 0u ? 2u : 0u) | ((raw & 1u) ? 0u : 4u) | ((raw & 8u) ? 0u : 8u);
    }
};
VGK_HD uint32_t* tb_miss_count(const GsswParams& P) { return reinterpret_cast<uint32_t*>(P.best + P.n_problems); }
VGK_HD uint32_t* tb_miss_list(const GsswParams& P) { return reinterpret_cast<uint32_t*>(P.best + P.n_problems + 1); }
VGK_HD uint64_t tb_best_entries(uint64_t n) { return n + 2u + (n + 1u) / 2u; }
VGK_HD void tb_miss_add(const GsswParams& P, uint32_t i) {
#if defined(__HIP_DEVICE_COMPILE__)
    const uint32_t k = atomicAdd(tb_miss_count(P), 1u);
#else
    const uint32_t k = (*tb_miss_count(P))++;
#endif
    tb_miss_list(P)[k] = i;
}
VGK_HD uint32_t* tb_bound_broken_count(const GsswParams& P) { return tb_miss_count(P) + 1; }
VGK_HD void tb_bound_broken(const GsswParams& P) {
#if defined(__HIP_DEVICE_COMPILE__)
    atomicAdd(tb_bound_broken_count(P), 1u);
#else
    ++*tb_bound_broken_count(P);
#endif
}
VGK_HD uint32_t refill_col0(const GsswParams& P, const ProbDesc& d, unsigned long long key, uint32_t& node0) {
    node0 = 0;
    const uint32_t S = (uint32_t)(key >> 40), c_e = 0xFFFFFu - (uint32_t)((key >> 20) & 0xFFFFFu), r_e = 0xFFFFFu - (uint32_t)(key & 0xFFFFFu);
    const uint32_t gx = P.go < P.ge ? P.go : P.ge;
    if (!S || !gx || r_e >= d.L || c_e >= d.R) return 0;
    const long long num = (long long)P.refill_m * (r_e + 1u) + d.bonus_start + d.bonus_end - (long long)S * P.scale - P.go;
    const unsigned long long span = (unsigned long long)r_e + (num < 0 ? 0ull : 1ull + (unsigned long long)num / gx);
    if (span >= c_e) return 0;
    const uint32_t col0 = (c_e - (uint32_t)span) & ~3u;
    if (!col0) return 0;
    const NodeRec* nodes = P.nodes + d.node_off;
    uint32_t begun = 0;
    for (uint32_t n = 0; n < d.n_nodes; ++n) {
        const NodeRec nr = nodes[n];
        if (nr.pinning || (n ? nr.n_pred != 1u || P.preds[nr.pred_begin] != n - 1u : nr.n_pred != 0u)) return 0;
        begun += nr.col_start < col0 ? 1u : 0u;
    }
    node0 = begun;
    return col0;
}
VGK_HD void refill_layout_one(const GsswParams& P, uint32_t w2) {
    const uint32_t M = *tb_miss_count(P), G = P.refill_G, gpw = 64u / G;
    const uint32_t n_pairs2 = (M + 1u) / 2u, n_waves2 = (n_pairs2 + gpw - 1u) / gpw;
    if (w2 == 0) P.refill_count[0] = n_waves2;
    if (w2 >= n_waves2) return;
    const uint32_t* list = tb_miss_list(P);
    ProbDesc* probs = const_cast<ProbDesc*>(P.probs);
    uint32_t* order = const_cast<uint32_t*>(P.order);
    WaveDesc* waves = const_cast<WaveDesc*>(P.waves);
    WaveDesc wd; wd.first_pair = P.refill_pair0 + w2 * gpw; wd.G = G; wd.pair_end = P.refill_pair0 + n_pairs2;
    uint32_t rmax = 0;
    for (uint32_t q = 0; q < gpw; ++q) for (uint32_t h = 0; h < 2u; ++h) {
        const uint32_t k = 2u * (w2 * gpw + q) + h;
        const uint32_t i = k < M ? list[k] : 0xffffffffu;
        if (w2 * gpw + q < n_pairs2) order[2u * (size_t)P.refill_pair0 + k] = i;
        if (i == 0xffffffffu) continue;
        ProbDesc& d = probs[i];
        uint32_t cols = d.R;
        d.col0 = 0; d.node0 = 0;
        if ((d.flags & 15u) == (uint32_t)VGK_GSSW_LOCAL) {
            const unsigned long long key = P.best[i];
            const uint32_t c_e = 0xFFFFFu - (uint32_t)((key >> 20) & 0xFFFFFu);
            if (c_e + 1u < cols) cols = c_e + 1u;
            if (P.refill_bound && (d.flags & VGK_GSSW_TRACEBACK)) d.col0 = refill_col0(P, d, key, d.node0);
        }
        rmax = cols - d.col0 > rmax ? cols - d.col0 : rmax;
        if (!(d.pad & 0x80000000u)) d.pad = 0x80000000u | (d.wave & 0xffffffu) | ((d.lane0 & 63u) << 24) | (((d.geom >> 16) & 1u) << 30);
        d.wave = P.refill_wave0 + w2; d.lane0 = q * G; d.geom = P.refill_K | (G << 8) | (h << 16);
// ... 32 lines not shown
```

vg_amd/csrc/pk16.hpp:

```cpp
#pragma once
#include <stdint.h>

#if defined(__HIPCC__)
#define VGK_HD __host__ __device__ __forceinline__
#else
#define VGK_HD inline
#endif

namespace vgk {

#if defined(__HIP_DEVICE_COMPILE__)
typedef unsigned short v2u16 __attribute__((ext_vector_type(2)));
static __device__ __forceinline__ v2u16 as_v(uint32_t x) { return __builtin_bit_cast(v2u16, x); }
static __device__ __forceinline__ uint32_t as_u(v2u16 x) { return __builtin_bit_cast(uint32_t, x); }
static __device__ __forceinline__ uint32_t pk_add(uint32_t a, uint32_t b) { return as_u(as_v(a) + as_v(b)); }
static __device__ __forceinline__ uint32_t pk_sub(uint32_t a, uint32_t b) { return as_u(as_v(a) - as_v(b)); }
static __device__ __forceinline__ uint32_t pk_subs(uint32_t a, uint32_t b) { return as_u(__builtin_elementwise_sub_sat(as_v(a), as_v(b))); }
static __device__ __forceinline__ uint32_t pk_max(uint32_t a, uint32_t b) { return as_u(__builtin_elementwise_max(as_v(a), as_v(b))); }
static __device__ __forceinline__ uint32_t pk_min(uint32_t a, uint32_t b) { return as_u(__builtin_elementwise_min(as_v(a), as_v(b))); }
static __device__ __forceinline__ uint32_t pk_mad(uint32_t a, uint32_t b, uint32_t c) { return as_u(as_v(a) * as_v(b) + as_v(c)); }
static __device__ __forceinline__ uint32_t byte_perm(uint32_t a, uint32_t b, uint32_t sel) { return __builtin_amdgcn_perm(a, b, sel); }
template <int M> static __device__ __forceinline__ uint32_t pk_mul_add_imm(uint32_t a, uint32_t c) {
    uint32_t r; asm("v_pk_mad_u16 %0, %1, %2, %3 op_sel_hi:[1,0,1]" : "=v"(r) : "v"(a), "n"(M), "v"(c)); return r; }
template <int C> static __device__ __forceinline__ uint32_t pk_mad_add_imm(uint32_t a, uint32_t b) {
    uint32_t r; asm("v_pk_mad_u16 %0, %1, %2, %3 op_sel_hi:[1,1,0]" : "=v"(r) : "v"(a), "s"(b), "n"(C)); return r; }
template <uint32_t MASK> static __device__ __forceinline__ uint32_t bit_select(uint32_t a, uint32_t b) {
    uint32_t r; asm("v_bfi_b32 %0, %1, %2, %3" : "=v"(r) : "s"(MASK), "v"(a), "v"(b)); return r; }
template <int N> static __device__ __forceinline__ uint32_t shl_or(uint32_t a, uint32_t c) {
    uint32_t r; asm("v_lshl_or_b32 %0, %1, %2, %3" : "=v"(r) : "v"(a), "n"(N), "v"(c)); return r; }
static __device__ __forceinline__ uint32_t pk_max3_f16(uint32_t a, uint32_t b, uint32_t c) {
    uint32_t r; asm("v_pk_maximum3_f16 %0, %1, %2, %3" : "=v"(r) : "v"(a), "v"(b), "v"(c)); return r; }
static __device__ __forceinline__ uint32_t pk_max_lo_into_hi(uint32_t a) {
    uint32_t r; asm("v_pk_max_u16 %0, %1, %1 op_sel:[0,0] op_sel_hi:[1,0]" : "=v"(r) : "v"(a)); return r; }
static __device__ __forceinline__ uint32_t pk_max_bhi(uint32_t a, uint32_t b) {
    uint32_t r; asm("v_pk_max_u16 %0, %1, %2 op_sel:[0,1] op_sel_hi:[1,1]" : "=v"(r) : "v"(a), "v"(b)); return r; }
static __device__ __forceinline__ uint32_t align16(uint32_t hi, uint32_t lo) { return __builtin_amdgcn_alignbit(hi, lo, 16); }
#else
static inline uint32_t pk_max_lo_into_hi(uint32_t a) { const uint32_t lo = a & 0xffffu, hi = a >> 16; return lo | ((hi > lo ? hi : lo) << 16); }
static inline uint32_t pk_max_bhi(uint32_t a, uint32_t b) { const uint32_t lo = a & 0xffffu, hi = a >> 16, t = b >> 16; return (lo > t ? lo : t) | ((hi > t ? hi : t) << 16); }
static inline uint32_t align16(uint32_t hi, uint32_t lo) { return (lo >> 16) | (hi << 16); }
template <uint32_t MASK> static inline uint32_t bit_select(uint32_t a, uint32_t b) { return (MASK & a) | (~MASK & b); }
template <int N> static inline uint32_t shl_or(uint32_t a, uint32_t c) { return (a << N) | c; }
static inline uint32_t pk_lo(uint32_t x) { return x & 0xffffu; }
static inline uint32_t pk_hi(uint32_t x) { return x >> 16; }
static inline uint32_t pk_mk(uint32_t lo, uint32_t hi) { return (lo & 0xffffu) | (hi << 16); }
static inline uint32_t pk_add(uint32_t a, uint32_t b) { return pk_mk(pk_lo(a) + pk_lo(b), pk_hi(a) + pk_hi(b)); }
static inline uint32_t pk_sub(uint32_t a, uint32_t b) { return pk_mk(pk_lo(a) - pk_lo(b), pk_hi(a) - pk_hi(b)); }
static inline uint32_t sat_sub16(uint32_t a, uint32_t b) { return a > b ? a - b : 0; }
static inline uint32_t pk_subs(uint32_t a, uint32_t b) { return pk_mk(sat_sub16(pk_lo(a), pk_lo(b)), sat_sub16(pk_hi(a), pk_hi(b))); }
static inline uint32_t pk_max(uint32_t a, uint32_t b) { return pk_mk(pk_lo(a) > pk_lo(b) ? pk_lo(a) : pk_lo(b), pk_hi(a) > pk_hi(b) ? pk_hi(a) : pk_hi(b)); }
static inline uint32_t pk_min(uint32_t a, uint32_t b) { return pk_mk(pk_lo(a) < pk_lo(b) ? pk_lo(a) : pk_lo(b), pk_hi(a) < pk_hi(b) ? pk_hi(a) : pk_hi(b)); }
static inline uint32_t pk_mad(uint32_t a, uint32_t b, uint32_t c) { return pk_mk(pk_lo(a) * pk_lo(b) + pk_lo(c), pk_hi(a) * pk_hi(b) + pk_hi(c)); }
static inline uint32_t pk_max3_f16(uint32_t a, uint32_t b, uint32_t c) { return pk_max(pk_max(a, b), c); }
template <int M> static inline uint32_t pk_mul_add_imm(uint32_t a, uint32_t c) { return pk_mad(a, (uint32_t)M * 0x00010001u, c); }
template <int C> static inline uint32_t pk_mad_add_imm(uint32_t a, uint32_t b) { return pk_mad(a, b, (uint32_t)C * 0x00010001u); }
static inline uint32_t byte_perm(uint32_t a, uint32_t b, uint32_t sel) {
    uint64_t src = ((uint64_t)a << 32) | b;
    uint32_t out = 0;
    for (int k = 0; k < 4; ++k) {
        uint32_t s = (sel >> (8 * k)) & 0xff, byte;
        if (s <= 7) byte = (uint32_t)(src >> (8 * s)) & 0xff;
        else if (s == 0x0c) byte = 0x00;
        else if (s >= 0x0d) byte = 0xff;
        else byte = 0;
        out |= byte << (8 * k);
    }
    return out;
}
#endif

VGK_HD uint32_t pk_add_nc(uint32_t a, uint32_t b) { return a + b; }
VGK_HD uint32_t pk_sub_nb(uint32_t a, uint32_t b) { return a - b; }

VGK_HD uint32_t set_lo(uint32_t x, uint32_t v) { return (x & 0xffff0000u) | (v & 0xffffu); }
VGK_HD uint32_t set_hi(uint32_t x, uint32_t v) { return (x & 0x0000ffffu) | (v << 16); }

}
```

vg_amd/csrc/vgk_api.cpp:

```cpp
#include <algorithm>
#include <chrono>
#include <cstdio>
#include <cstdlib>
#include <cstring>
#include <memory>
#include <mutex>
#include <new>
#include <string>
#include <vector>
#include "backend.hpp"
#include "ctx.hpp"
#include "host_parallel.hpp"

#include "batch.hpp"
#include "gssw_wide.hpp"

extern "C" {

int vgk_abi_version(void) { return VGK_ABI_VERSION; }

const char* vgk_strerror(int code) {
    switch (code) {
        case VGK_OK: return "ok";
        case VGK_EINVAL: return "invalid argument";
// ... 264 lines not shown
            }
            col = nr.col_end;
        }
        for (uint32_t c = d.col_off + col; c & 3u; ++c) colinfo[c] = (uint8_t)CI_INVALID;
    });

    lap("pass3");
    GsswParams& P = b->P;
    int rc;
    std::unique_lock<std::mutex> lk(ctx->mu);
    b->lane = (std::getenv("VGAMD_ONE_STREAM") ? 0 : (int)(ctx->batch_seq++ & 1u));
    auto fail = [&](int code) { vgk_batch* t = hb.release(); if (lk.owns_lock()) lk.unlock(); ctx->be->sync_side(); vgk_batch_free(t); return code; };
    auto issue_uploads = [&]() -> int {
        for (const vgk_batch::Upload& u : b->uploads) { const int e = ctx->be->upload_side(u.dst, u.src, u.bytes); if (e) return e; }
        b->uploads.clear();
        return VGK_OK;
    };
    if ((rc = to_device(b, colinfo, n_cols + 8, P.colinfo))) return fail(rc);
    if ((rc = to_device(b, reads, n_reads, P.reads, 8))) return fail(rc);
    if ((rc = to_device(b, prof, n_prof, P.prof, 4))) return fail(rc);
    if ((rc = to_device(b, nodes, n_nodes, P.nodes))) return fail(rc);
    if ((rc = to_device(b, preds, n_preds, P.preds, 1))) return fail(rc);
    lk.unlock();
    if ((rc = issue_uploads())) return fail(rc);
    lap("arenas");
    auto gkey = [&](uint32_t i) { return ((probs[i].geom & 0xffu) << 8) | ((probs[i].geom >> 8) & 0xffu); };
    std::vector<uint32_t> idx(n);
    {
        auto pass = [&](const uint32_t* src, uint32_t* dst, auto key) {
            constexpr uint32_t SLICES = 64, MAX_RANGE = 8192;
            uint32_t lo_k = 0xffffffffu, hi_k = 0;
            if (n >= 65536) {
                std::vector<uint32_t> mn(SLICES, 0xffffffffu), mx(SLICES, 0);
                parallel_tasks(SLICES, [&](uint32_t sl) {
                    const uint64_t a0 = (uint64_t)n * sl / SLICES, a1 = (uint64_t)n * (sl + 1) / SLICES;
                    uint32_t a = 0xffffffffu, b2 = 0;
                    for (uint64_t k = a0; k < a1; ++k) { const uint32_t v = key(src ? src[k] : (uint32_t)k); a = std::min(a, v); b2 = std::max(b2, v); }
                    mn[sl] = a; mx[sl] = b2;
                });
                for (uint32_t sl = 0; sl < SLICES; ++sl) { lo_k = std::min(lo_k, mn[sl]); hi_k = std::max(hi_k, mx[sl]); }
            }
            if (n >= 65536 && hi_k - lo_k < MAX_RANGE) {
                const uint32_t range = hi_k - lo_k + 1;
                std::vector<uint32_t> hist((size_t)SLICES * range, 0u);
                auto each_slice = [&](auto body) { parallel_tasks(SLICES, body); };
                each_slice([&](uint32_t sl) {
                    uint32_t* h = hist.data() + (size_t)sl * range;
                    const uint64_t a0 = (uint64_t)n * sl / SLICES, a1 = (uint64_t)n * (sl + 1) / SLICES;
                    for (uint64_t k = a0; k < a1; ++k) ++h[key(src ? src[k] : (uint32_t)k) - lo_k];
                });
                uint32_t at = 0;
                for (uint32_t v = 0; v < range; ++v)
                    for (uint32_t sl = 0; sl < SLICES; ++sl) { uint32_t& c = hist[(size_t)sl * range + v]; const uint32_t cnt = c; c = at; at += cnt; }
                each_slice([&](uint32_t sl) {
                    uint32_t* h = hist.data() + (size_t)sl * range;
                    const uint64_t a0 = (uint64_t)n * sl / SLICES, a1 = (uint64_t)n * (sl + 1) / SLICES;
                    for (uint64_t k = a0; k < a1; ++k) { const uint32_t i = src ? src[k] : (uint32_t)k; dst[h[key(i) - lo_k]++] = i; }
                });
                return;
            }
            std::vector<uint32_t> count(65537, 0u);
            for (uint32_t k = 0; k < n; ++k) ++count[key(src ? src[k] : k) + 1];
            for (uint32_t k = 0; k < 65536; ++k) count[k + 1] += count[k];
            for (uint32_t k = 0; k < n; ++k) { const uint32_t i = src ? src[k] : k; dst[count[key(i)]++] = i; }
        };
        std::vector<uint32_t> tmp(n);
        pass(nullptr, tmp.data(), [&](uint32_t i) { return 0xffffu - std::min<uint32_t>(probs[i].R, 0xffffu); });
        pass(tmp.data(), idx.data(), gkey);
    }
    lap("sort");
    struct Bucket { uint32_t s0, s1, K, G, pair0, pair1, wave0; };
    std::vector<Bucket> buckets;
    std::vector<FillLaunch>& launches = b->launches;
    uint32_t n_pairs = 0, n_waves = 0;
    for (uint32_t s0 = 0; s0 < n;) {
        const uint32_t gk = gkey(idx[s0]);
        uint32_t lo = s0, hi = n;
        while (hi - lo > 1) { const uint32_t mid = lo + (hi - lo) / 2; if (gkey(idx[mid]) == gk) lo = mid; else hi = mid; }
        const uint32_t s1 = hi, K = gk >> 8, G = gk & 0xffu, gpw = 64 / G;
        Bucket bk{s0, s1, K, G, n_pairs, n_pairs + (s1 - s0 + 1) / 2, n_waves};
        if (launches.empty() || launches.back().K != K) launches.push_back(FillLaunch{K, n_waves, 0});
        n_pairs = bk.pair1; n_waves += (bk.pair1 - bk.pair0 + gpw - 1) / gpw;
        launches.back().wave_count = n_waves - launches.back().wave_begin;
        buckets.push_back(bk);
        s0 = s1;
    }
    uint32_t local_tb = 0;
    for (uint32_t i = 0; i < n; ++i) local_tb += (problems[i].flags & (15u | VGK_GSSW_TRACEBACK)) == (uint32_t)(VGK_GSSW_LOCAL | VGK_GSSW_TRACEBACK) ? 1u : 0u;
    const bool fused_env = std::getenv("VGAMD_FUSED_TRACEBACK") && std::atoi(std::getenv("VGAMD_FUSED_TRACEBACK"));
    const bool walk2 = !fused_env && n >= 1024 && 2ull * local_tb >= n && !std::getenv("VGAMD_WALK_ONE_PASS");
    bool spec = walk2 && b->want_tb && buckets.size() == 1 && launches.size() == 1 && default_tb_mode(fused_env ? 1 : 0, !all.far) == TB_CODES && !std::getenv("VGAMD_NO_SPEC_FILL");
    uint64_t refill_slot = 0;
    if (spec) { uint32_t rmax_all = 0; for (uint32_t i = 0; i < n; ++i) rmax_all = std::max(rmax_all, probs[i].R);
                refill_slot = tb_wave_dwords(rmax_all + buckets[0].G - 1, buckets[0].K); }
    std::vector<uint32_t> order((size_t)(spec ? 4 : 2) * n_pairs, 0xffffffffu);
    std::vector<WaveDesc> waves((size_t)(spec ? 2 : 1) * n_waves);
    parallel_for(n_waves, [&](uint32_t w, unsigned) {
        size_t bi = 0;
        while (bi + 1 < buckets.size() && buckets[bi + 1].wave0 <= w) ++bi;
        const Bucket& bk = buckets[bi];
        const uint32_t gpw = 64 / bk.G, pw = bk.pair0 + (w - bk.wave0) * gpw;
        WaveDesc wd{};
        wd.first_pair = pw; wd.G = bk.G; wd.pair_end = bk.pair1;
        uint32_t rmax = 0;
        for (uint32_t q = 0; q < gpw && pw + q < bk.pair1; ++q)
            for (uint32_t h = 0; h < 2; ++h) {
                const uint32_t k = bk.s0 + 2 * (pw + q - bk.pair0) + h;
                const uint32_t i = k < bk.s1 ? idx[k] : 0xffffffffu;
                order[2 * (size_t)(pw + q) + h] = i;
                if (i == 0xffffffffu) continue;
                rmax = std::max(rmax, probs[i].R);
                probs[i].wave = w; probs[i].lane0 = q * bk.G; probs[i].geom = bk.K | (bk.G << 8) | (h << 16);
            }
        wd.n_steps = rmax ? rmax + bk.G - 1 : 0;
        wd.tb_off = b->want_tb ? tb_wave_dwords(wd.n_steps, bk.K) : 0;
        waves[w] = wd;
    });
    uint64_t tb_dwords = 0;
    for (uint32_t w = 0; w < n_waves; ++w) { WaveDesc& wd = waves[w]; const uint64_t size = wd.tb_off; wd.tb_off = tb_dwords; tb_dwords += size; b->wave_steps += wd.n_steps; }
    if (spec && (uint64_t)n_waves * refill_slot > tb_dwords + tb_dwords / 2) spec = false;
    if (spec) tb_dwords = (uint64_t)n_waves * refill_slot;

    lap("waves");
    lk.lock();
    if ((rc = to_device(b, (const ProbDesc*)probs, (size_t)n, P.probs))) return fail(rc);
    if ((rc = to_device(b, waves, P.waves))) return fail(rc);
    if ((rc = to_device(b, order, P.order, 2))) return fail(rc);
    if ((rc = dev_alloc(b, (size_t)scratch_words + 16, P.scratch))) return fail(rc);
    if ((rc = dev_alloc(b, (size_t)tb_dwords + 4, P.tb))) return fail(rc);
    if ((rc = dev_alloc(b, (size_t)tb_best_entries(n), P.best))) return fail(rc);
    if ((rc = dev_alloc(b, (size_t)n + 1, P.results))) return fail(rc);
    if ((rc = dev_alloc(b, (size_t)ops_total + 1, P.ops))) return fail(rc);
    P.spec_fill = 0; P.wave_limit = nullptr; P.refill_count = nullptr; P.refill_wave0 = P.refill_pair0 = P.refill_G = P.refill_K = 0; P.refill_slot = 0;
    if (spec) {
        if ((rc = dev_alloc(b, (size_t)4, P.refill_count))) return fail(rc);
        P.spec_fill = 1; P.refill_wave0 = n_waves; P.refill_pair0 = n_pairs; P.refill_G = buckets[0].G; P.refill_K = buckets[0].K; P.refill_slot = refill_slot;
    }
    lap("allocs");
    lk.unlock();
    if ((rc = issue_uploads())) return fail(rc);
    P.wave_begin = 0; P.wave_count = 0; P.K = 0;
    P.n_problems = n; P.n_pairs = n_pairs; P.n_waves = n_waves;
    const uint32_t S = ctx->scale;
    for (int q = 0; q < 6; ++q) P.prof4[q] = ctx->prof4[q] * S;
    P.bias = ctx->bias * S; P.go = ctx->sc.gap_open * S; P.ge = ctx->sc.gap_extend * S; P.bonus = ctx->sc.full_length_bonus * (int32_t)S;
    P.scale = S; P.xoff = XOFF * S;
    P.want_tb = b->want_tb ? 1 : 0;
    P.fused = 0;
    if (const char* e = std::getenv("VGAMD_FUSED_TRACEBACK")) P.fused = std::atoi(e) ? 1 : 0;
    P.dbg = std::getenv("VGAMD_TB_DBG") ? std::atoi(std::getenv("VGAMD_TB_DBG")) : 0; P.tb_mode = default_tb_mode(P.fused, !all.far);
    P.walk_passes = walk2 && !P.fused ? 2 : 1;
    if (P.walk_passes != 2 || P.tb_mode != TB_CODES) P.spec_fill = 0;
    set_refill_bound(P, ctx);
    P.key3 = 0;
    if (P.spec_fill) {
        uint32_t longest = 0; bool xdrop = false;
        for (uint32_t i = 0; i < n; ++i) { longest = std::max(longest, probs[i].L); xdrop = xdrop || (problems[i].flags & 15u) == (uint32_t)VGK_XDROP_PINNED; }
        P.key3 = gssw_key3_ok(S, ctx->has_qa, xdrop, longest, (uint32_t)std::max(0, ctx->max_score), (uint32_t)std::max(0, ctx->max_bonus)) && !std::getenv("VGAMD_NO_KEY3") ? 1u : 0u;
    }
    std::memcpy(P.matrix, ctx->sc.matrix, 25);
    b->ops_total = ops_total;
    if ((rc = ctx->be->sync_side())) return fail(rc);
    lap("uploads");
    *out = hb.release();
    return VGK_OK;
} catch (const std::bad_alloc&) { return VGK_ENOMEM; } catch (...) { return VGK_EINVAL; }

static void observe_speculation(vgk_batch* b) {
    if (!b->ran || !b->ran_spec || b->spec_observed || !b->P.refill_count) return;
    b->spec_observed = true;
    uint32_t refilled = 0;
    if (b->ctx->be->download_fetch(&refilled, b->P.refill_count, sizeof refilled) != VGK_OK) return;
    b->ctx->spec.observe(b->P.n_waves ? (double)refilled / (double)b->P.n_waves : 0.0, b->spec_probe);
}

int vgk_gssw_run(vgk_batch* b) try {
    if (!b) return VGK_EINVAL;
    std::lock_guard<std::mutex> lk(b->ctx->mu);
    if (!b->done) b->done = b->ctx->be->event_create();
    GsswParams P = b->P;
    if (b->P.spec_fill) {
        if (b->ran && b->ran_spec && !b->spec_observed && b->ctx->be->event_done(b->done)) observe_speculation(b);
        bool probe = false;
        const bool speculate = b->ctx->spec.decide(&probe);
        b->spec_probe = probe;
        if (!speculate) {
            P.spec_fill = 0; P.wave_limit = nullptr;
            P.restore_probs = b->probs_displaced ? 1 : 0;
            b->probs_displaced = false;
        } else b->probs_displaced = true;
        b->ran_spec = speculate; b->spec_observed = !speculate;
    }
    const int rc = b->ctx->be->run_gssw_on(b->lane, P, b->launches.data(), (uint32_t)b->launches.size(), true, b->done);
    if (rc == VGK_OK) b->ran = true;
    return rc;
} catch (const std::bad_alloc&) { return VGK_ENOMEM; } catch (...) { return VGK_EINVAL; }

int vgk_batch_sync(vgk_batch* b) try {
    if (!b) return VGK_EINVAL;
    return b->done ? b->ctx->be->event_wait(b->done) : b->ctx->be->sync();
} catch (const std::bad_alloc&) { return VGK_ENOMEM; } catch (...) { return VGK_EINVAL; }

static int fetch_packed_on_device(vgk_batch* b, vgk_result* results, vgk_op* ops, size_t ops_cap, size_t* ops_written) {
    vgk_ctx* ctx = b->ctx; Backend* be = ctx->be.get();
    const uint32_t n = b->n;
    if (!n) return VGK_EUNSUPPORTED;
    const uint32_t blocks = (n + Backend::OPS_SCAN_BLOCK - 1) / Backend::OPS_SCAN_BLOCK;
    std::vector<vgk_ctx::Pooled> mine;
    auto take = [&](uint64_t bytes) -> void* { std::lock_guard<std::mutex> lk(ctx->mu); uint64_t got = 0; void* p = ctx->dev_take(bytes, got); if (p) mine.push_back({p, got}); return p; };
    struct GiveBack { vgk_ctx* ctx; std::vector<vgk_ctx::Pooled>& v; ~GiveBack() { ctx->be->sync_fetch(); std::lock_guard<std::mutex> lk(ctx->mu); for (auto& q : v) ctx->dev_give(q.p, q.bytes); } } give_back{ctx, mine};
    uint32_t* offs = (uint32_t*)take((uint64_t)n * 4);
    uint32_t* sums = (uint32_t*)take(((uint64_t)blocks + 8) * 4);
    if (!offs || !sums) return VGK_ENOMEM;
    uint64_t total = 0;
    int rc = be->ops_offsets(b->P.results, n, offs, sums, &total);
    if (rc) return rc;
    if (total && (!ops || total > ops_cap || !b->want_tb)) return VGK_EUNSUPPORTED;
    vgk_result* out_res = (vgk_result*)take((uint64_t)n * sizeof(vgk_result));
    vgk_op* out_ops = (vgk_op*)take((total + 1) * sizeof(vgk_op));
    if (!out_res || !out_ops) return VGK_ENOMEM;
    if ((rc = be->ops_gather(b->P.results, b->P.ops, n, offs, sums, out_res, out_ops))) return rc;
    struct StagingLease {
        vgk_ctx* ctx; std::unique_ptr<vgk_ctx::Staging> s;
        ~StagingLease() { if (s) ctx->staging_release(std::move(s)); }
    } lease{ctx, ctx->staging_acquire()};
    const uint64_t res_bytes = (uint64_t)n * sizeof(vgk_result), ops_bytes = total * sizeof(vgk_op);
    uint8_t* stage = (uint8_t*)lease.s->get(5, res_bytes + ops_bytes);
    if (!stage) return VGK_ENOMEM;
    if ((rc = be->download_fetch(stage, out_res, res_bytes))) return rc;
    if (ops_bytes && (rc = be->download_fetch(stage + res_bytes, out_ops, ops_bytes))) return rc;
    auto copy_out = [](void* dst, const uint8_t* src, uint64_t bytes) {
        const uint64_t chunk = 16384;
        parallel_for((uint32_t)((bytes + chunk - 1) / chunk), [&](uint32_t c, unsigned) {
            const uint64_t at = (uint64_t)c * chunk;
            std::memcpy((uint8_t*)dst + at, src + at, (size_t)std::min(chunk, bytes - at));
        });
    };
    copy_out(results, stage, res_bytes);
    if (ops_bytes) copy_out(ops, stage + res_bytes, ops_bytes);
    b->alg_bytes = b->in_bytes + 16ull * n + 2ull * total + b->tb_cells;
    if (ops_written) *ops_written = (size_t)total;
    return VGK_OK;
}

static void translate_extension_results(const vgk_batch* b, vgk_result* results, vgk_op* ops) {
    parallel_chunks(b->n, [&](uint32_t lo, uint32_t hi, uint32_t) {
        for (uint32_t i = lo; i < hi; ++i) {
            vgk_result& r = results[i];
            if (r.status != VGK_OK) continue;
            if (b->ext_count[i] == WIN_EXT_DUMMY) { r.score = 0; r.n_ops = 0; r.end_node = r.end_offset = r.end_read = -1; r.first_offset = 0; continue; }
            const uint32_t* nodes = b->ext_nodes.data() + b->ext_off[i]; const uint32_t cnt = b->ext_count[i];
            if (r.end_node >= 0 && (uint32_t)r.end_node < cnt) r.end_node = (int32_t)nodes[r.end_node];
            if (ops) for (uint32_t k = 0; k < r.n_ops; ++k) { vgk_op& o = ops[r.ops_begin + k]; if (o.node < cnt) o.node = nodes[o.node]; }
        }
    });
}

static int gssw_fetch_impl(vgk_batch* b, vgk_result* results, vgk_op* ops, size_t ops_cap, size_t* ops_written);
int vgk_gssw_fetch(vgk_batch* b, vgk_result* results, vgk_op* ops, size_t ops_cap, size_t* ops_written) try {
    const int rc = gssw_fetch_impl(b, results, ops, ops_cap, ops_written);
    if ((rc == VGK_OK || rc == VGK_EOPS) && b && !b->ext_count.empty()) translate_extension_results(b, results, ops);
    return rc;
} catch (const std::bad_alloc&) { return VGK_ENOMEM; } catch (...) { return VGK_EINVAL; }

static int gssw_fetch_impl(vgk_batch* b, vgk_result* results, vgk_op* ops, size_t ops_cap, size_t* ops_written) {
    if (!b || !results) return VGK_EINVAL;
    if (!b->ran) { int rc = vgk_gssw_run(b); if (rc) return rc; }
    { int rc = b->done ? b->ctx->be->event_wait(b->done) : b->ctx->be->sync(); if (rc) return rc; }
    int rc = b->ctx->be->fetch_after(b->done);
    if (rc) return rc;
    { std::lock_guard<std::mutex> lk(b->ctx->mu); if (b->ran_spec && !b->spec_observed) observe_speculation(b); }
    rc = fetch_packed_on_device(b, results, ops, ops_cap, ops_written);
    if (rc != VGK_EUNSUPPORTED) return rc;
    std::lock_guard<std::mutex> lk(b->ctx->mu);
    rc = b->ctx->be->download(results, b->P.results, (size_t)b->n * sizeof(vgk_result));
    if (rc) return rc;
    struct StagingLease {
        vgk_ctx* ctx; std::unique_ptr<vgk_ctx::Staging> s;
        ~StagingLease() { if (s) ctx->staging_release(std::move(s)); }
    } lease{b->ctx, nullptr};
    const vgk_op* all = nullptr;
    if (b->want_tb && b->ops_total) {
        lease.s = b->ctx->staging_acquire();
        vgk_op* buf = (vgk_op*)lease.s->get(5, (uint64_t)b->ops_total * sizeof(vgk_op));
        if (!buf) return VGK_ENOMEM;
        rc = b->ctx->be->download(buf, b->P.ops, (size_t)b->ops_total * sizeof(vgk_op));
        if (rc) return rc;
        all = buf;
    }
    size_t w = 0; uint64_t alg = 0;
    std::vector<uint32_t> src(b->n);
    std::vector<ProbDesc> fetched;
    const ProbDesc* descs = b->probs;
    if (!descs && b->n) {
        fetched.resize(b->n);
        if ((rc = b->ctx->be->download(fetched.data(), b->P.probs, (size_t)b->n * sizeof(ProbDesc)))) return rc;
        descs = fetched.data();
    }
    for (uint32_t i = 0; i < b->n; ++i) {
        vgk_result& r = results[i];
        const ProbDesc& d = descs[i];
        src[i] = r.ops_begin;
        if (r.status == VGK_OK && r.n_ops) {
            if (!ops || w + r.n_ops > ops_cap) { r.status = VGK_EOPS; r.n_ops = 0; r.ops_begin = (uint32_t)w; continue; }
            r.ops_begin = (uint32_t)w; w += r.n_ops;
        } else { r.n_ops = 0; r.ops_begin = (uint32_t)w; }
        alg += 16 + 2ull * r.n_ops + ((d.flags & VGK_GSSW_TRACEBACK) ? (uint64_t)d.L * d.R : 0);
    }
    if (all) parallel_for(b->n, [&](uint32_t i, unsigned) {
        const vgk_result& r = results[i];
        if (r.status == VGK_OK && r.n_ops) std::memcpy(ops + r.ops_begin, all + src[i], (size_t)r.n_ops * sizeof(vgk_op));
    });
    b->alg_bytes = b->in_bytes + alg;
    if (ops_written) *ops_written = w;
    return VGK_OK;
}

static uint64_t problem_device_bytes(const vgk_gssw_problem& p) {
    uint64_t R = 0;
    for (uint32_t v = 0; v < p.graph.n_nodes; ++v) R += p.graph.node_len[v];
    const uint64_t rows = ((uint64_t)p.read_len + 24) / 4 * 4 + 4;
    const uint64_t bytes = rows * (R + 64) / 2 + 16 * (p.read_len + R) + (4 * rows + 64) * p.graph.n_nodes + 512;
    return bytes + bytes / 8;
}

static int problem_limit_status(const vgk_ctx* ctx, const vgk_gssw_problem& p) {
    if (p.read_len == 0 || !p.read || p.graph.n_nodes == 0) return VGK_EINVAL;
    const uint32_t mode = p.flags & 15u;
    const bool xdrop = mode == VGK_XDROP_PINNED;
    const uint32_t rows = p.read_len + (xdrop ? 1u : 0u);
    if (rows > 1024) return VGK_ETOOLONG;
    if ((int64_t)rows * std::max(ctx->max_score, 0) + 2 * (int64_t)ctx->max_bonus > 2046) return VGK_EUNSUPPORTED;
    if (xdrop && (int64_t)p.read_len * std::max(ctx->max_score, 0) + ctx->max_bonus >= (int64_t)XOFF) return VGK_EUNSUPPORTED;
    return VGK_OK;
}

int vgk_gssw_align(vgk_ctx* ctx, const vgk_gssw_problem* problems, uint32_t n,
                   vgk_result* results, vgk_op* ops, size_t ops_cap, size_t* ops_written) try {
    if (!ctx || (!problems && n) || !results) return VGK_EINVAL;
    uint64_t budget = ctx->be->memory_bytes();
    budget = budget ? budget / 2 : (8ull << 30);
    if (const char* e = std::getenv("VGAMD_MAX_BATCH_BYTES")) budget = std::strtoull(e, nullptr, 10);
    std::vector<uint32_t> runnable, wide; runnable.reserve(n);
    for (uint32_t i = 0; i < n; ++i) {
        const int st = problem_limit_status(ctx, problems[i]);
        if (st == VGK_OK) runnable.push_back(i);
        else if (st == VGK_ETOOLONG || st == VGK_EUNSUPPORTED) wide.push_back(i);
        else { std::memset(&results[i], 0, sizeof results[i]); results[i].status = st; }
    }
    const bool all = runnable.size() == n;
    std::vector<vgk_gssw_problem> sub_problems; std::vector<vgk_result> sub_results;
    size_t w_total = 0;
    size_t begin = 0;
    while (begin < runnable.size()) {
        size_t end = begin; uint64_t bytes = 0;
        while (end < runnable.size()) {
            const uint64_t pb = problem_device_bytes(problems[runnable[end]]);
            if (end > begin && bytes + pb > budget) break;
            bytes += pb; ++end;
        }
        const uint32_t m = (uint32_t)(end - begin);
        const vgk_gssw_problem* batch_problems = problems + begin;
        vgk_result* batch_results = results + begin;
        if (!all) {
            sub_problems.resize(m); sub_results.resize(m);
            for (uint32_t k = 0; k < m; ++k) sub_problems[k] = problems[runnable[begin + k]];
            batch_problems = sub_problems.data(); batch_results = sub_results.data();
        }
        vgk_batch* b = nullptr;
        int rc = vgk_gssw_pack(ctx, batch_problems, m, 0, &b);
        if (rc == VGK_ENOMEM && m > 1) {
            budget = std::max<uint64_t>(bytes / 2, 1);
            continue;
        }
        if (rc) return rc;
        rc = vgk_gssw_run(b);
        size_t w = 0;
        if (!rc) rc = vgk_gssw_fetch(b, batch_results, ops ? ops + w_total : nullptr, ops_cap - w_total, &w);
        vgk_batch_free(b);
        if (rc) return rc;
        for (uint32_t k = 0; k < m; ++k) {
            batch_results[k].ops_begin += (uint32_t)w_total;
            if (!all) results[runnable[begin + k]] = batch_results[k];
        }
        w_total += w;
        begin = end;
    }
    if (!wide.empty()) {
        const int rc = wide_align(ctx, problems, wide.data(), (uint32_t)wide.size(), results, ops, ops_cap, &w_total);
        if (rc) return rc;
    }
    if (ops_written) *ops_written = w_total;
    return VGK_OK;
} catch (const std::bad_alloc&) { return VGK_ENOMEM; } catch (...) { return VGK_EINVAL; }

double vgk_batch_kernel_ms(vgk_batch* b, int which) {
    if (!b) return 0.0;
    std::lock_guard<std::mutex> lk(b->ctx->mu);
    if (which == 0 || which == 1 || which == 2) return b->ctx->be->last_ms_on(b->lane, which);
    if (which == 3) return b->P.spec_fill && b->ran_spec ? b->ctx->be->last_ms_on(b->lane, 12) : 0.0;
    return b->ctx->be->last_ms_on(b->lane, 0) + b->ctx->be->last_ms_on(b->lane, 1);
}
uint64_t vgk_batch_cells(vgk_batch* b) { return b ? b->cells : 0; }
uint64_t vgk_batch_alg_bytes(vgk_batch* b) {
    if (!b) return 0;
    if (b->alg_bytes) return b->alg_bytes;
    uint64_t alg = b->in_bytes;
    if (!b->probs) return alg + 16ull * b->n + b->tb_cells;
    for (uint32_t i = 0; i < b->n; ++i) { const ProbDesc& d = b->probs[i]; alg += 16 + ((d.flags & VGK_GSSW_TRACEBACK) ? (uint64_t)d.L * d.R : 0); }
    return alg;
}
uint64_t vgk_batch_device_bytes(vgk_batch* b) { return b ? b->dev_bytes : 0; }
uint64_t vgk_batch_wave_steps(vgk_batch* b) { return b ? b->wave_steps : 0; }
extern "C" int vgk_batch_refill_stats(vgk_batch* b, uint64_t out[5]) try {
    if (!b || !out) return VGK_EINVAL;
    for (int k = 0; k < 5; ++k) out[k] = 0;
    { const int rc = vgk_batch_sync(b); if (rc) return rc; }
    std::lock_guard<std::mutex> lk(b->ctx->mu);
    if (!b->ran || !b->ran_spec || !b->P.refill_count) return VGK_OK;
    Backend* be = b->ctx->be.get();
    uint32_t n_waves2 = 0, counters[2] = {0, 0};
    int rc = be->download(&n_waves2, b->P.refill_count, sizeof n_waves2);
    if (!rc) rc = be->download(counters, tb_miss_count(b->P), sizeof counters);
    if (rc) return rc;
    const uint32_t missed = std::min(counters[0], b->n);
    std::vector<WaveDesc> waves(n_waves2); std::vector<uint32_t> list(missed); std::vector<ProbDesc> probs(b->n);
    if (n_waves2 && (rc = be->download(waves.data(), b->P.waves + b->P.refill_wave0, waves.size() * sizeof(WaveDesc)))) return rc;
    if (missed && (rc = be->download(list.data(), tb_miss_list(b->P), list.size() * sizeof(uint32_t)))) return rc;
    if (missed && (rc = be->download(probs.data(), b->P.probs, probs.size() * sizeof(ProbDesc)))) return rc;
    out[0] = n_waves2; out[2] = missed; out[4] = counters[1];
    for (const WaveDesc& wd : waves) out[1] += wd.n_steps;
    for (uint32_t i : list) if (i < b->n && probs[i].col0) ++out[3];
    return VGK_OK;
} catch (const std::bad_alloc&) { return VGK_ENOMEM; } catch (...) { return VGK_EINVAL; }
int      vgk_batch_lane(vgk_batch* b) { return b ? b->lane : 0; }
int      vgk_batch_speculated(vgk_batch* b) { if (!b) return 0; std::lock_guard<std::mutex> lk(b->ctx->mu); return b->ran && b->ran_spec ? 1 : 0; }
int      vgk_set_speculation(vgk_ctx* ctx, int mode) {
    if (!ctx || mode < 0 || mode > 2) return VGK_EINVAL;
    std::lock_guard<std::mutex> lk(ctx->mu);
    ctx->spec.mode = mode;
    return VGK_OK;
}
int      vgk_speculation_state(vgk_ctx* ctx, uint64_t counters[4], double* last_miss) {
    if (!ctx) return VGK_EINVAL;
    std::lock_guard<std::mutex> lk(ctx->mu);
    if (counters) { counters[0] = ctx->spec.observed; counters[1] = ctx->spec.turned_off; counters[2] = ctx->spec.turned_on; counters[3] = ctx->spec.on ? 0 : ctx->spec.interval; }
    if (last_miss) *last_miss = ctx->spec.last_miss;
    return ctx->spec.on ? 1 : 0;
}

}
```

vg_amd/csrc/window_api.cpp:

```cpp
#include <algorithm>
#include <atomic>
#include <chrono>
#include <cstdio>
#include <cstdlib>
#include <cstring>
#include <memory>
#include <mutex>
#include <new>
#include <vector>
#include "batch.hpp"
#include "dgraph.hpp"
#include "host_parallel.hpp"


namespace {

inline int ref_code(char ch) {
    switch (ch) { case 'A': return 0; case 'C': return 1; case 'G': return 2; case 'T': return 3; default: return 4; }
}

struct Lap {
    std::chrono::steady_clock::time_point t0 = std::chrono::steady_clock::now(); const bool on = std::getenv("VGAMD_TIMING") != nullptr;
    void operator()(const char* what) {
        if (!on) return;
// ... 117 lines not shown
    } temp_guard{ctx, temp};
    auto fail = [&](int code) { vgk_batch* t = hb.release(); ctx->be->sync_side(); vgk_batch_free(t); return code; };
    auto take_temp = [&](uint64_t bytes) -> void* { uint64_t got = 0; void* p = ctx->dev_take(bytes ? bytes : 16, got); if (p) temp.push_back({p, got}); return p; };
    auto take_keep = [&](uint64_t bytes) -> void* { uint64_t got = 0; void* p = ctx->dev_take(bytes ? bytes : 16, got); if (p) { b->dev.push_back({p, got}); b->dev_bytes += bytes; } return p; };

    bool near_chain = false;
    if (!on_device && !extensions && !dg->far_prefix.empty()) {
        std::atomic<bool> far{false};
        const std::vector<uint32_t>& fp = dg->far_prefix; const uint32_t gn = dg->g.n_nodes;
        parallel_chunks(n, [&](uint32_t lo, uint32_t hi, uint32_t) {
            for (uint32_t i = lo; i < hi; ++i) {
                const vgk_window_problem& w = problems[i];
                if (w.n_nodes < 2 || w.first_node >= gn || w.n_nodes > gn - w.first_node) continue;
                if (fp[w.first_node + w.n_nodes] != fp[w.first_node + 1]) { far.store(true, std::memory_order_relaxed); break; }
            }
        });
        near_chain = !far.load();
    }
    const uint32_t n1 = n + 1;
    const uint32_t waves_cap = n / 2 + WIN_BUCKETS + 1;
    WinParams W{};
    W.g = dg->g; W.n = n; W.raw_bytes = reads_bytes; W.ops_per_problem = ops_per_problem;
    W.forced_k = forced_k;
    if (const char* e = std::getenv("VGAMD_ROWS_PER_LANE")) W.forced_k = (uint32_t)std::atoi(e);
    W.max_score = ctx->max_score; W.max_bonus = ctx->max_bonus; W.scale = ctx->scale; W.bonus = ctx->sc.full_length_bonus;
    W.n_waves_cap = waves_cap;
    void* tmp = nullptr; size_t tmp_bytes = be->win_tmp_bytes(n, waves_cap);
    int rc;
    rc = VGK_OK;
    uint64_t ext_nodes_total = 0;
    {
        std::lock_guard<std::mutex> lk(ctx->mu);
        W.problems = on_device ? problems : (const vgk_window_problem*)take_temp((uint64_t)n * sizeof(vgk_window_problem));
        W.raw_reads = on_device ? (const uint8_t*)reads : (const uint8_t*)take_temp(reads_bytes + 8);
        W.sizes = (uint32_t*)take_temp((uint64_t)WIN_COLS * n1 * 4); W.offs = (uint32_t*)take_temp((uint64_t)WIN_COLS * n1 * 4);
        W.key = (uint32_t*)take_temp((uint64_t)n * 4); W.idx = (uint32_t*)take_temp((uint64_t)n * 4);
        W.key_sorted = (uint32_t*)take_temp((uint64_t)n * 4); W.idx_sorted = (uint32_t*)take_temp((uint64_t)n * 4);
        W.totals = (WinTotals*)take_temp(sizeof(WinTotals));
        W.bucket_first = (uint32_t*)take_temp(sizeof(uint32_t) * WIN_BUCKETS); W.buckets = (WinBucket*)take_temp(sizeof(WinBucket) * WIN_BUCKETS);
        W.wave_tb = (unsigned long long*)take_temp(((uint64_t)waves_cap + 1) * 8);
        tmp = take_temp(tmp_bytes);
        b->lane = (std::getenv("VGAMD_ONE_STREAM") ? 0 : (int)(ctx->batch_seq++ & 1u));
        W.probs = (ProbDesc*)take_keep((uint64_t)std::max<uint32_t>(n, 1u) * sizeof(ProbDesc));
        if (extensions) {
            ext_nodes_total = n ? (uint64_t)extensions[n - 1].kept_off + problems[n - 1].n_nodes : 0;
            W.ext = (const WinExt*)take_temp((uint64_t)std::max<uint32_t>(n, 1u) * sizeof(WinExt));
            W.kept = (WinKept*)take_temp((ext_nodes_total + 1) * sizeof(WinKept)); W.ext_count = (uint32_t*)take_temp((uint64_t)std::max<uint32_t>(n, 1u) * 4);
            W.kept_node = (uint32_t*)take_temp((ext_nodes_total + 1) * 4);
            if (!W.ext || !W.kept || !W.ext_count || !W.kept_node) rc = VGK_ENOMEM;
        }
        if (!W.problems || !W.raw_reads || !W.sizes || !W.offs || !W.key || !W.idx || !W.key_sorted || !W.idx_sorted || !W.totals ||
            !W.bucket_first || !W.buckets || !W.wave_tb || !tmp || !W.probs) rc = VGK_ENOMEM;
    }
    if (rc) return fail(rc);
    lap("device buffers");
    {
        WinTotals zero{}; zero.first_bad = ~0ull;
        WinTotals* tz = (WinTotals*)lease.s->get(2, sizeof(WinTotals));
        if (!tz) return fail(VGK_ENOMEM);
        *tz = zero;
        if ((rc = be->upload_side(W.totals, tz, sizeof(WinTotals)))) return fail(rc);
    }
    auto staged_upload = [&](int slot, void* dst, const void* src, uint64_t bytes) -> int {
        if (!bytes) return VGK_OK;
        uint8_t* st = (uint8_t*)lease.s->get(slot, bytes);
        if (!st) return VGK_ENOMEM;
        const uint64_t SLICE = 16ull << 20, PIECE = 256ull << 10;
        for (uint64_t at = 0; at < bytes; at += SLICE) {
            const uint64_t len = std::min(SLICE, bytes - at);
            parallel_tasks((uint32_t)((len + PIECE - 1) / PIECE), [&](uint32_t c) {
                const uint64_t o = at + (uint64_t)c * PIECE;
                std::memcpy(st + o, (const uint8_t*)src + o, (size_t)std::min(PIECE, at + len - o));
            });
            const int e = be->upload_side((uint8_t*)dst + at, st + at, len);
            if (e) return e;
        }
        return VGK_OK;
    };
    if (!on_device && (rc = staged_upload(1, (void*)W.problems, problems, (uint64_t)n * sizeof(vgk_window_problem)))) return fail(rc);
    if (extensions && (rc = staged_upload(3, (void*)W.ext, extensions, (uint64_t)n * sizeof(WinExt)))) return fail(rc);
    lap("problems staged");
    if ((rc = be->win_stage1(W, tmp, tmp_bytes))) return fail(rc);
    if (!on_device && (rc = staged_upload(0, (void*)W.raw_reads, reads, reads_bytes))) return fail(rc);
    lap("reads staged");
    WinTotals T;
    if ((rc = be->download_side(&T, W.totals, sizeof T))) return fail(rc);
    lap("stage 1 (sizes)");
    if (T.first_bad != ~0ull) return fail(-(int)(T.first_bad & 0xffu));
    for (uint32_t k = 0; k < WIN_COLS; ++k) if (T.tot[k] >= (1ull << 32)) return fail(VGK_ETOOBIG);
    if (extensions && n) {
        uint32_t* st_nodes = (uint32_t*)lease.s->get(4, (ext_nodes_total + 1) * 4); uint32_t* st_count = (uint32_t*)lease.s->get(6, (uint64_t)n * 4);
        if (!st_nodes || !st_count) return fail(VGK_ENOMEM);
        if ((rc = be->download_side(st_count, W.ext_count, (size_t)n * 4))) return fail(rc);
        if ((rc = be->download_side(st_nodes, W.kept_node, (size_t)ext_nodes_total * 4))) return fail(rc);
        b->ext_count.assign(st_count, st_count + n); b->ext_nodes.assign(st_nodes, st_nodes + ext_nodes_total);
        b->ext_off.resize((size_t)n + 1);
        for (uint32_t i = 0; i < n; ++i) b->ext_off[i] = extensions[i].kept_off;
        b->ext_off[n] = (uint32_t)ext_nodes_total;
        lap("extension nodes");
    }
    b->want_tb = T.want_tb != 0; b->cells = T.cells; b->tb_cells = T.tb_cells; b->in_bytes = T.in_bytes;
    W.want_tb = b->want_tb ? 1 : 0;
    uint8_t* colinfo; uint8_t* rd; NodeRec* nodes; uint32_t* preds; WaveDesc* waves; uint32_t* order;
    {
        std::lock_guard<std::mutex> lk(ctx->mu);
        colinfo = (uint8_t*)take_keep(T.tot[WS_COLS] + 8); rd = (uint8_t*)take_keep(T.tot[WS_READS] + 8);
        nodes = (NodeRec*)take_keep((T.tot[WS_NODES] + 1) * sizeof(NodeRec)); preds = (uint32_t*)take_keep((T.tot[WS_PREDS] + 1) * 4);
        waves = (WaveDesc*)take_keep((uint64_t)waves_cap * sizeof(WaveDesc)); order = (uint32_t*)take_keep(((uint64_t)waves_cap * 4 + 4) * 4);
        rc = dev_alloc(b, (size_t)T.tot[WS_SCRATCH] + 16, P.scratch);
        if (!rc) rc = dev_alloc(b, (size_t)tb_best_entries(n), P.best);
        if (!rc) rc = dev_alloc(b, (size_t)n + 1, P.results);
        if (!rc) rc = dev_alloc(b, (size_t)T.tot[WS_OPS] + 1, P.ops);
        if (!rc && (!colinfo || !rd || !nodes || !preds || !waves || !order)) rc = VGK_ENOMEM;
    }
    if (rc) return fail(rc);
    W.colinfo = colinfo; W.reads = rd; W.nodes = nodes; W.preds = preds; W.waves = waves; W.order = order;
    if ((rc = be->fill_side(colinfo + T.tot[WS_COLS], (int)CI_INVALID, 8))) return fail(rc);
    if ((rc = be->win_stage2(W, tmp, tmp_bytes))) return fail(rc);
    if ((rc = be->download_side(&T, W.totals, sizeof T))) return fail(rc);
    lap("stage 2 (order, waves, arenas)");
    if (T.n_waves > waves_cap || T.n_launches > 4) return fail(VGK_EINVAL);
    uint32_t local_tb = 0;
    if (!on_device) for (uint32_t i = 0; i < n; ++i) local_tb += (problems[i].flags & (15u | VGK_GSSW_TRACEBACK)) == (uint32_t)(VGK_GSSW_LOCAL | VGK_GSSW_TRACEBACK) ? 1u : 0u;
    const bool walk2 = !on_device && n >= 1024 && 2ull * local_tb >= n && !std::getenv("VGAMD_WALK_ONE_PASS");
    bool spec = walk2 && b->want_tb && T.n_launches == 1 && T.n_buckets == 1 && T.first_G && default_tb_mode(0, near_chain) == TB_CODES && 2ull * T.n_waves <= waves_cap &&
                !std::getenv("VGAMD_NO_SPEC_FILL");
    uint64_t refill_slot = 0, tb_dwords = T.tb_dwords;
    if (spec) {
        refill_slot = tb_wave_dwords(T.max_steps, T.launch_K[0]);
        if ((uint64_t)T.n_waves * refill_slot > T.tb_dwords + T.tb_dwords / 2) spec = false;
        else tb_dwords = (uint64_t)T.n_waves * refill_slot;
    }
    P.spec_fill = 0; P.wave_limit = nullptr; P.refill_count = nullptr; P.refill_wave0 = P.refill_pair0 = P.refill_G = P.refill_K = 0; P.refill_slot = 0;
    {
        std::lock_guard<std::mutex> lk(ctx->mu);
        rc = dev_alloc(b, (size_t)tb_dwords + 4, P.tb);
        if (!rc && spec) rc = dev_alloc(b, (size_t)4, P.refill_count);
    }
    if (rc) return fail(rc);
    if (spec) { P.spec_fill = 1; P.refill_wave0 = T.n_waves; P.refill_pair0 = T.n_pairs; P.refill_G = T.first_G; P.refill_K = T.launch_K[0]; P.refill_slot = refill_slot; }
    for (uint32_t k = 0; k < T.n_launches; ++k) b->launches.push_back(FillLaunch{T.launch_K[k], T.launch_begin[k], T.launch_count[k]});
    P.probs = W.probs; P.colinfo = colinfo; P.reads = rd; P.prof = nullptr; P.nodes = nodes; P.preds = preds; P.waves = waves; P.order = order;
    P.wave_begin = 0; P.wave_count = 0; P.K = 0;
    P.n_problems = n; P.n_pairs = T.n_pairs; P.n_waves = T.n_waves;
    const uint32_t S = ctx->scale;
    for (int q = 0; q < 6; ++q) P.prof4[q] = ctx->prof4[q] * S;
    P.bias = ctx->bias * S; P.go = ctx->sc.gap_open * S; P.ge = ctx->sc.gap_extend * S; P.bonus = ctx->sc.full_length_bonus * (int32_t)S;
    P.scale = S; P.xoff = XOFF * S;
    P.want_tb = b->want_tb ? 1 : 0;
    P.fused = 0; P.dbg = std::getenv("VGAMD_TB_DBG") ? std::atoi(std::getenv("VGAMD_TB_DBG")) : 0; P.tb_mode = default_tb_mode(0, near_chain);
    P.walk_passes = walk2 ? 2 : 1;
    if (P.walk_passes != 2 || P.tb_mode != TB_CODES) P.spec_fill = 0;
    set_refill_bound(P, ctx);
    P.key3 = 0;
    if (P.spec_fill) {
        uint32_t longest = 0; bool xdrop = false;
        for (uint32_t i = 0; i < n; ++i) { longest = std::max(longest, problems[i].read_len); xdrop = xdrop || (problems[i].flags & 15u) == (uint32_t)VGK_XDROP_PINNED; }
        P.key3 = gssw_key3_ok(S, ctx->has_qa, xdrop, longest, (uint32_t)std::max(0, ctx->max_score), (uint32_t)std::max(0, ctx->max_bonus)) && !std::getenv("VGAMD_NO_KEY3") ? 1u : 0u;
    }
    std::memcpy(P.matrix, ctx->sc.matrix, 25);
    b->ops_total = T.tot[WS_OPS]; b->wave_steps = T.wave_steps;
    lap("done");
    *out = hb.release();
    return VGK_OK;
} catch (const std::bad_alloc&) { return VGK_ENOMEM; } catch (...) { return VGK_EINVAL; }

int vgk_gssw_pack_windows(vgk_ctx* ctx, const vgk_dgraph* dg, const char* reads, size_t reads_bytes,
                          const vgk_window_problem* problems, uint32_t n, uint32_t ops_per_problem, vgk_batch** out) try {
    return vgk_pack_windows_impl(ctx, dg, reads, reads_bytes, problems, n, ops_per_problem, out, false, 0, nullptr);
} catch (const std::bad_alloc&) { return VGK_ENOMEM; } catch (...) { return VGK_EINVAL; }

int vgk_gssw_pack_extensions(vgk_ctx* ctx, const vgk_dgraph* dg, const char* reads, size_t reads_bytes,
                             const vgk_extension_problem* problems, uint32_t n, uint32_t ops_per_problem, vgk_batch** out) try {
    if (!ctx || !dg || dg->ctx != ctx || !out || (!problems && n) || (!reads && reads_bytes)) return VGK_EINVAL;
    if (!dg->g.succ_off) return VGK_EUNSUPPORTED;
    std::vector<vgk_window_problem> win(n); std::vector<WinExt> ext(n);
    uint64_t at = 0;
    for (uint32_t i = 0; i < n; ++i) {
        const vgk_extension_problem& p = problems[i];
        vgk_window_problem& w = win[i]; WinExt& x = ext[i];
        w.read_off = p.read_off; w.read_len = p.read_len; w.flags = p.flags; w.first_node = p.first_node; w.n_nodes = p.n_nodes; w.max_gap_length = p.max_gap_length; w.reserved = 0;
        x.start_node = p.start_node; x.start_offset = p.start_offset; x.query_offset = p.query_offset; x.leftward = p.leftward ? 1u : 0u; x.kept_off = (uint32_t)at; x.pad = 0;
        at += p.n_nodes;
        if (at >= (1ull << 32) - 16) return VGK_ETOOBIG;
    }
    return vgk_pack_windows_impl(ctx, dg, reads, reads_bytes, win.data(), n, ops_per_problem, out, false, 0, ext.data());
} catch (const std::bad_alloc&) { return VGK_ENOMEM; } catch (...) { return VGK_EINVAL; }

}
```

Measured before the change: 71.83 million.

## Offset DP rows by a floor constant to drop saturating subtracts in key3 fill

Adds a row offset (floor) to all H/E/F values in the speculative key3 S8 fill kernel. Every score then stays above the gap and bias penalties, so saturating packed subtracts become plain non-borrowing subtracts and a max3 against the floor. Scratch stores and seeds strip and re-add the offset, and the key computation folds the offset into its constant. This makes a new kernel template variant and risks overflow if the range check in gssw_row_offset is wrong.

```diff
diff --git a/include/vgk_engine.h b/include/vgk_engine.h
--- a/include/vgk_engine.h
+++ b/include/vgk_engine.h
@@ -30,6 +30,8 @@
 
 int vgk_batch_refill_stats(vgk_batch* batch, uint64_t out[5]);
 
+uint32_t vgk_batch_row_offset(vgk_batch* batch);
+
 #ifdef __cplusplus
 }
 #endif
diff --git a/vg_amd/capi.py b/vg_amd/capi.py
--- a/vg_amd/capi.py
+++ b/vg_amd/capi.py
@@ -999,6 +999,11 @@
         self.eng._check(f(self.h, out), "vgk_batch_refill_stats")
         return dict(zip(("waves", "steps", "missed", "bounded", "broken"), (int(v) for v in out)))
 
+    def row_offset(self):
+        f = self.eng.lib.vgk_batch_row_offset
+        f.restype = ctypes.c_uint32; f.argtypes = [ctypes.c_void_p]
+        return int(f(self.h))
+
     def speculated(self):
         self.eng.lib.vgk_batch_speculated.argtypes = [ctypes.c_void_p]
         return bool(self.eng.lib.vgk_batch_speculated(self.h))
diff --git a/vg_amd/csrc/backend_hip.hip b/vg_amd/csrc/backend_hip.hip
--- a/vg_amd/csrc/backend_hip.hip
+++ b/vg_amd/csrc/backend_hip.hip
@@ -45,7 +45,7 @@
     }
 };
 
-template <int K, bool S8, bool REWALK, bool CODES = true, bool KEY3 = false, bool NOKEY = false>
+template <int K, bool S8, bool REWALK, bool CODES = true, bool KEY3 = false, bool NOKEY = false, bool OFFS = false>
 __global__ __launch_bounds__(256, (K <= 16 ? 4 : 3)) void gssw_fill_kernel(const GsswParams P) {
     constexpr uint32_t REC = (K + 3) / 4;
     __shared__ __attribute__((aligned(16))) uint32_t stage_lds[4][REWALK ? 64u * TB_BND_CHUNK * 2u : (TB_TILE > 1 ? TbStage<K>::DWORDS : 256u)];
@@ -59,7 +59,7 @@
     __shared__ uint32_t pb_lds[4][64 * K];
     s.PBL = (typename Lane<K>::lds_u32*)(pb_lds[threadIdx.x >> 6] + lane);
 #endif
-    lane_init<K, NOKEY ? 1 : 0>(s, P, wd, lane);
+    lane_init<K, NOKEY ? 1 : 0, OFFS ? 1 : 0>(s, P, wd, lane);
     asm volatile("" : "+v"(s.one));
     uint32_t* tb = P.want_tb ? P.tb : nullptr;
     TbStage<K> stage{stage_lds[threadIdx.x >> 6]};
@@ -76,17 +76,17 @@
         for (; t < steady_from; ++t) {
             if ((t & 3u) == 0) lane_prefetch(s, P, t);
             const uint32_t rh = from_lane_above(s.out_h), rf = from_lane_above(s.out_f), ri = from_lane_above(s.info);
-            lane_step<K, S8, false, KEY3>(s, P, t, rh, rf, ri, nullptr, nullptr);
+            lane_step<K, S8, false, KEY3, false, false, OFFS ? 1 : 0>(s, P, t, rh, rf, ri, nullptr, nullptr);
         }
         for (; t < steady_to; ++t) {
             if ((t & 3u) == 0) lane_prefetch(s, P, t);
             const uint32_t rh = from_lane_above(s.out_h), rf = from_lane_above(s.out_f), ri = from_lane_above(s.info);
-            lane_step<K, S8, false, KEY3, false, true>(s, P, t, rh, rf, ri, nullptr, nullptr);
+            lane_step<K, S8, false, KEY3, false, true, OFFS ? 1 : 0>(s, P, t, rh, rf, ri, nullptr, nullptr);
         }
         for (; t < wd.n_steps; ++t) {
             if ((t & 3u) == 0) lane_prefetch(s, P, t);
             const uint32_t rh = from_lane_above(s.out_h), rf = from_lane_above(s.out_f), ri = from_lane_above(s.info);
-            lane_step<K, S8, false, KEY3>(s, P, t, rh, rf, ri, nullptr, nullptr);
+            lane_step<K, S8, false, KEY3, false, false, OFFS ? 1 : 0>(s, P, t, rh, rf, ri, nullptr, nullptr);
         }
     }
     for (uint32_t t = 0; CODES && t < wd.n_steps; ++t) {
@@ -96,7 +96,7 @@
         const uint32_t ri = from_lane_above(s.info);
         if constexpr (!CODES) {
         } else if constexpr (REWALK) {
-            lane_step<K, S8, false>(s, P, t, rh, rf, ri, nullptr, nullptr);
+            lane_step<K, S8, false, false, false, false, 0>(s, P, t, rh, rf, ri, nullptr, nullptr);
             if (tb) {
                 uint32_t* st = stage_lds[threadIdx.x >> 6] + lane * (TB_BND_CHUNK * 2u);
                 const uint32_t slot = (t ^ lane) & (TB_BND_CHUNK - 1u);
@@ -114,10 +114,10 @@
                 lane_store_checkpoint<K>(s, P, wd, t, lane);
             }
         } else if constexpr (TB_TILE > 1) {
-            lane_step<K, S8, true, false, NOKEY>(s, P, t, rh, rf, ri, tb ? stage.slot_a(t, lane) : nullptr, stage.slot_b(t, lane));
+            lane_step<K, S8, true, false, NOKEY, false, 0>(s, P, t, rh, rf, ri, tb ? stage.slot_a(t, lane) : nullptr, stage.slot_b(t, lane));
             if (tb && ((t % TB_TILE) == TB_TILE - 1u || t + 1u == wd.n_steps)) stage.flush(tb + tb_tile_base(wd.tb_off, t, REC), lane);
         } else
-            lane_step<K, S8, true, false, NOKEY>(s, P, t, rh, rf, ri, tb ? tb + tb_dword(wd.tb_off, t, lane, REC, 0) : nullptr, tb ? tb + tb_dword(wd.tb_off, t, lane, REC, 4) : nullptr);
+            lane_step<K, S8, true, false, NOKEY, false, 0>(s, P, t, rh, rf, ri, tb ? tb + tb_dword(wd.tb_off, t, lane, REC, 0) : nullptr, tb ? tb + tb_dword(wd.tb_off, t, lane, REC, 4) : nullptr);
     }
     if constexpr (NOKEY) return;
     if (REWALK || !CODES || !P.fused) {
@@ -1327,7 +1327,8 @@
         const dim3 grid((p.wave_count + 3) / 4), block(256);
         const bool s8 = p.scale == 8, re = p.tb_mode == TB_REWALK;
         if (p.spec_fill == 1) {
-            if (s8 && p.key3) hipLaunchKernelGGL((gssw_fill_kernel<K, true, false, false, true>), grid, block, 0, stream, p);
+            if (s8 && p.key3 && p.row_off) hipLaunchKernelGGL((gssw_fill_kernel<K, true, false, false, true, false, true>), grid, block, 0, stream, p);
+            else if (s8 && p.key3) hipLaunchKernelGGL((gssw_fill_kernel<K, true, false, false, true>), grid, block, 0, stream, p);
             else if (s8) hipLaunchKernelGGL((gssw_fill_kernel<K, true, false, false>), grid, block, 0, stream, p); else hipLaunchKernelGGL((gssw_fill_kernel<K, false, false, false>), grid, block, 0, stream, p);
             return VGK_OK;
         }
diff --git a/vg_amd/csrc/gssw_device.hpp b/vg_amd/csrc/gssw_device.hpp
--- a/vg_amd/csrc/gssw_device.hpp
+++ b/vg_amd/csrc/gssw_device.hpp
@@ -96,6 +96,7 @@
     uint32_t scale;
     uint32_t xoff;
     int8_t   matrix[25];
+    uint32_t row_off;
 };
 
 VGK_HD uint32_t rep2(uint32_t x) { return (x & 0xffffu) * 0x00010001u; }
@@ -161,8 +162,9 @@
     const uint32_t keep = (1u << (8u * (R - t))) - 1u;
     return (w & keep) | (none & ~keep);
 }
-template <int K, int SECOND = -1>
+template <int K, int SECOND = -1, int OFS = -1>
 VGK_HD void lane_init(Lane<K>& s, const GsswParams& P, const WaveDesc& wd, uint32_t lane_id) {
+    const uint32_t floor2 = (OFS > 0 || (OFS < 0 && P.key3 && P.spec_fill == 1)) ? rep2(P.row_off) : 0u;
     const uint32_t q = lane_id / wd.G;
     s.g = lane_id - q * wd.G;
     s.Lpad = wd.G * K;
@@ -195,9 +197,9 @@
         uint32_t pa = 0, pb = 0;
         if (row < s.LA) pa = poA != 0xffffffffu ? P.prof[poA + row] : pw.of_row(P.reads[roA + row]) + 0x01010101u * row_bonus(s.bsA, s.beA, row, s.LA);
         if (row < s.LB) pb = poB != 0xffffffffu ? P.prof[poB + row] : pw.of_row(P.reads[roB + row]) + 0x01010101u * row_bonus(s.bsB, s.beB, row, s.LB);
-        s.PA[m] = pa; s.set_pb(m, pb); s.H[m] = 0; s.E[m] = 0;
-    }
-    s.out_h = 0; s.out_f = 0; s.info = CI_INVALID2; s.prev_rh = 0;
+        s.PA[m] = pa; s.set_pb(m, pb); s.H[m] = floor2; s.E[m] = floor2;
+    }
+    s.out_h = floor2; s.out_f = floor2; s.info = CI_INVALID2; s.prev_rh = floor2;
     s.best_lo = s.best_hi = 0; s.step_lo = s.step_hi = 0;
     s.nodeA = SECOND != 0 ? n0A - 1u : 0xffffffffu; s.nodeB = SECOND != 0 ? n0B - 1u : 0xffffffffu;
     s.one = 0x00010001u;
@@ -226,13 +228,14 @@
 #endif
 
 template <int HALF, int K>
-VGK_HD void seed_from_scratch(Lane<K>& s, const GsswParams& P, uint32_t prob, uint32_t node, uint32_t& diag0) {
+VGK_HD void seed_from_scratch(Lane<K>& s, const GsswParams& P, uint32_t prob, uint32_t node, uint32_t& diag0, uint32_t floor2) {
     const ProbDesc& d = P.probs[prob];
     const NodeRec& nr = P.nodes[d.node_off + node];
     const uint32_t keep = HALF == 0 ? 0xffff0000u : 0x0000ffffu;
-#pragma unroll
-    for (int m = 0; m < K; ++m) { s.H[m] &= keep; s.E[m] &= keep; }
-    diag0 &= keep;
+    const uint32_t fl = floor2 & ~keep;
+#pragma unroll
+    for (int m = 0; m < K; ++m) { s.H[m] = (s.H[m] & keep) | fl; s.E[m] = (s.E[m] & keep) | fl; }
+    diag0 = (diag0 & keep) | fl;
     if (nr.n_pred == 0 && (d.flags & 15u) == VGK_XDROP_PINNED) {
 #pragma unroll
         for (int m = 0; m <= K; ++m) {
@@ -257,25 +260,25 @@
 #pragma unroll
         for (int m = 0; m < K; ++m) {
             const uint32_t v = scratch_load(base + m);
-            s.H[m] = pk_max(s.H[m], HALF == 0 ? (v & 0xffffu) : (v << 16));
-            s.E[m] = pk_max(s.E[m], HALF == 0 ? (v >> 16) : (v & 0xffff0000u));
+            s.H[m] = pk_max(s.H[m], (HALF == 0 ? (v & 0xffffu) : (v << 16)) + fl);
+            s.E[m] = pk_max(s.E[m], (HALF == 0 ? (v >> 16) : (v & 0xffff0000u)) + fl);
         }
         if (s.g > 0) {
             const uint32_t v = scratch_load(base - 1);
-            diag0 = pk_max(diag0, HALF == 0 ? (v & 0xffffu) : (v << 16));
+            diag0 = pk_max(diag0, (HALF == 0 ? (v & 0xffffu) : (v << 16)) + fl);
         }
     }
 }
 
 template <int HALF, int K>
-VGK_HD void store_to_scratch(const Lane<K>& s, const GsswParams& P, uint32_t prob, uint32_t node) {
+VGK_HD void store_to_scratch(const Lane<K>& s, const GsswParams& P, uint32_t prob, uint32_t node, uint32_t floor2) {
     const ProbDesc& d = P.probs[prob];
     const NodeRec& nr = P.nodes[d.node_off + node];
     uint32_t* base = P.scratch + d.scratch_off + (uint32_t)nr.slot * s.Lpad + s.g * K;
 #pragma unroll
     for (int m = 0; m < K; ++m) {
-        uint32_t h = HALF == 0 ? (s.H[m] & 0xffffu) : (s.H[m] >> 16);
-        uint32_t e = HALF == 0 ? (s.E[m] & 0xffffu) : (s.E[m] >> 16);
+        uint32_t h = (HALF == 0 ? (s.H[m] & 0xffffu) : (s.H[m] >> 16)) - (floor2 & 0xffffu);
+        uint32_t e = (HALF == 0 ? (s.E[m] & 0xffffu) : (s.E[m] >> 16)) - (floor2 & 0xffffu);
         base[m] = h | (e << 16);
     }
 }
@@ -303,23 +306,53 @@
 VGK_HD bool gssw_key3_ok(uint32_t scale, bool quality_adjusted, bool any_xdrop, uint32_t longest_read, uint32_t max_score, uint32_t max_bonus) {
     return scale == 8u && !quality_adjusted && !any_xdrop && (uint64_t)longest_read * max_score + 2ull * max_bonus <= 990ull;
 }
+VGK_HD uint32_t gssw_row_offset(uint32_t scale, uint32_t go, uint32_t ge, uint32_t bias) {
+    uint32_t a = go > ge ? go : ge; a = bias > a ? bias : a;
+    return scale * 990u + a + 255u < 0x7c00u ? a : 0u;
+}
+#ifndef VGK_DIAG_ADD3
+#define VGK_DIAG_ADD3 1
+#endif
+VGK_HD uint32_t diag_unbias(uint32_t d, uint32_t sb, uint32_t nb) {
+#if VGK_DIAG_ADD3
+    (void)pk_sub_nb(pk_add_nc(d, sb), 0u - nb);
+    return d + sb + nb;
+#else
+    return pk_sub_nb(pk_add_nc(d, sb), nb);
+#endif
+}
 constexpr uint32_t KEY_SHIFT = 5, KEY_LOW = 31;
 
 template <int K, int M, bool REFN, bool S8, bool TB>
-VGK_HD uint32_t row_diag(const Lane<K>& s, const GsswParams& P, uint32_t sel, uint32_t bias2, bool nA, bool nB, uint32_t d) {
+VGK_HD uint32_t row_diag(const Lane<K>& s, const GsswParams& P, uint32_t sel, uint32_t bias2, bool nA, bool nB, uint32_t d, bool ofs) {
     uint32_t sb = byte_perm(s.pb(M), s.PA[M], sel);
     if (REFN) {
         const uint32_t row = s.g * K + M;
         if (nA) sb = set_lo(sb, row < s.LA ? P.bias + row_bonus(s.bsA, s.beA, row, s.LA) : 0u);
         if (nB) sb = set_hi(sb, row < s.LB ? P.bias + row_bonus(s.bsB, s.beB, row, s.LB) : 0u);
     }
+    if (ofs) return diag_unbias(d, sb, bias2);
     return pk_subs(pk_add_nc(d, sb), (TB && S8) ? bias2 - 0x00040004u : bias2);
 }
 template <int K, int M, bool REFN, bool S8, bool TB, bool K3, bool NK>
 VGK_HD void lane_row(Lane<K>& s, const GsswParams& P, uint32_t sel, uint32_t bias2, uint32_t go2, uint32_t ge2,
-                     bool nA, bool nB, uint32_t& f, uint32_t& d, uint32_t* acc, uint32_t& ck) {
+                     bool nA, bool nB, uint32_t& f, uint32_t& d, uint32_t* acc, uint32_t& ck, bool ofs) {
     const uint32_t t4 = d;
-    if constexpr (M + 1 < K) d = row_diag<K, M + 1, REFN, S8, TB>(s, P, sel, bias2, nA, nB, s.H[M]);
+    if constexpr (M + 1 < K) d = row_diag<K, M + 1, REFN, S8, TB>(s, P, sel, bias2, nA, nB, s.H[M], ofs);
+    if constexpr (!TB && S8 && K3) {
+        if (ofs) {
+            const uint32_t floor2 = rep2(P.row_off);
+            const uint32_t e = s.E[M];
+            const uint32_t h = pk_max3_f16(t4, e, f);
+            const uint32_t gg = pk_sub_nb(h, go2);
+            const uint32_t en = pk_max3_f16_u(gg, pk_sub_nb(e, ge2), floor2), fn = pk_max3_f16_u(gg, pk_sub_nb(f, ge2), floor2);
+            const uint32_t key = pk_mul_imm_add_u<1 << (KEY_SHIFT - 3)>(h, rep2((uint32_t)((int)KEY_LOW - M) - (P.row_off << (KEY_SHIFT - 3))));
+            if constexpr ((M & 1) == 0) { if constexpr (M + 1 < K) acc[0] = key; else ck = M == 0 ? key : pk_max(ck, key); }
+            else ck = M == 1 ? pk_max(acc[0], key) : pk_max3_f16(ck, acc[0], key);
+            s.H[M] = h; s.E[M] = en; f = fn;
+            return;
+        }
+    }
     if constexpr (!TB) {
         const uint32_t e = s.E[M];
         const uint32_t h = (S8 && VGK_H_MAX3) ? pk_max3_f16(t4, e, f) : pk_max(pk_max(t4, e), f);
@@ -369,26 +402,31 @@
 
 template <int K, int M, bool REFN, bool S8, bool TB, bool K3, bool NK>
 VGK_HD void lane_rows_from(Lane<K>& s, const GsswParams& P, uint32_t sel, uint32_t bias2, uint32_t go2, uint32_t ge2,
-                           bool nA, bool nB, uint32_t& f, uint32_t& d, uint32_t* acc, uint32_t& ck) {
-    lane_row<K, M, REFN, S8, TB, K3, NK>(s, P, sel, bias2, go2, ge2, nA, nB, f, d, acc, ck);
-    if constexpr (M + 1 < K) lane_rows_from<K, M + 1, REFN, S8, TB, K3, NK>(s, P, sel, bias2, go2, ge2, nA, nB, f, d, acc, ck);
+                           bool nA, bool nB, uint32_t& f, uint32_t& d, uint32_t* acc, uint32_t& ck, bool ofs) {
+    lane_row<K, M, REFN, S8, TB, K3, NK>(s, P, sel, bias2, go2, ge2, nA, nB, f, d, acc, ck, ofs);
+    if constexpr (M + 1 < K) lane_rows_from<K, M + 1, REFN, S8, TB, K3, NK>(s, P, sel, bias2, go2, ge2, nA, nB, f, d, acc, ck, ofs);
 }
 
 template <int K, bool REFN, bool S8, bool TB, bool K3, bool NK>
 VGK_HD void lane_rows(Lane<K>& s, const GsswParams& P, uint32_t sel, uint32_t diag0, uint32_t rf,
-                      bool nA, bool nB, uint32_t* acc, uint32_t& colkey) {
+                      bool nA, bool nB, uint32_t* acc, uint32_t& colkey, bool ofs) {
     uint32_t bias2 = rep2(P.bias), go2 = rep2(P.go), ge2 = rep2(P.ge);
+    if (ofs && VGK_DIAG_ADD3) bias2 = 0u - bias2;
 #if defined(__HIP_DEVICE_COMPILE__)
     if (REFN) asm volatile("" : "+v"(sel), "+v"(bias2), "+v"(go2), "+v"(ge2));
 #endif
-    uint32_t f = rf, d = row_diag<K, 0, REFN, S8, TB>(s, P, sel, bias2, nA, nB, diag0), ck = 0;
-    lane_rows_from<K, 0, REFN, S8, TB, K3, NK>(s, P, sel, bias2, go2, ge2, nA, nB, f, d, acc, ck);
+    uint32_t f = rf, d = row_diag<K, 0, REFN, S8, TB>(s, P, sel, bias2, nA, nB, diag0, ofs), ck = 0;
+    lane_rows_from<K, 0, REFN, S8, TB, K3, NK>(s, P, sel, bias2, go2, ge2, nA, nB, f, d, acc, ck, ofs);
     s.out_h = s.H[K - 1]; s.out_f = f;
     colkey = ck;
 }
 
-template <int K, bool S8, bool TB, bool RE, bool K3 = false, bool NK = false, bool AV = false>
+template <bool S8, bool TB, bool K3, int OFS>
+VGK_HD bool offset_rows(const GsswParams& P) { return S8 && !TB && K3 && (OFS > 0 || (OFS < 0 && P.row_off != 0u)); }
+template <int K, bool S8, bool TB, bool RE, bool K3 = false, bool NK = false, bool AV = false, int OFS = -1>
 VGK_HD void lane_column(Lane<K>& s, const GsswParams& P, uint32_t t, uint32_t rh, uint32_t rf, uint32_t rinfo, uint32_t* tb_a, uint32_t* tb_b) {
+    const bool ofs = offset_rows<S8, TB, K3, OFS>(P);
+    const uint32_t floor2 = ofs ? rep2(P.row_off) : 0u;
     s.info = rinfo;
     const uint32_t ia = rinfo & 0xffu, ib = (rinfo >> 16) & 0xffu;
     const bool vA = AV || !(ia & CI_INVALID), vB = AV || !(ib & CI_INVALID);
@@ -397,13 +435,13 @@
         if (vA && (ia & CI_NODE_START)) s.nodeA += 1;
         if (vB && (ib & CI_NODE_START)) s.nodeB += 1;
         if (rinfo & (CI_SEED_SLOW * 0x00010001u)) {
-            if (vA && (ia & CI_SEED_SLOW)) seed_from_scratch<0, K>(s, P, s.probA, s.nodeA, diag0);
-            if (vB && (ib & CI_SEED_SLOW)) seed_from_scratch<1, K>(s, P, s.probB, s.nodeB, diag0);
+            if (vA && (ia & CI_SEED_SLOW)) seed_from_scratch<0, K>(s, P, s.probA, s.nodeA, diag0, floor2);
+            if (vB && (ib & CI_SEED_SLOW)) seed_from_scratch<1, K>(s, P, s.probB, s.nodeB, diag0, floor2);
         }
         const uint32_t sel = (rinfo & 0x00030003u) | 0x0c040c00u;
         uint32_t acc[(K + 3) / 4], colkey;
-        if (rinfo & 0x00040004u) { const bool nA = (ia & CI_BASE_MASK) == 4, nB = (ib & CI_BASE_MASK) == 4; lane_rows<K, true, S8, TB, K3, NK>(s, P, sel, diag0, rf, nA, nB, acc, colkey); }
-        else          lane_rows<K, false, S8, TB, K3, NK>(s, P, sel, diag0, rf, false, false, acc, colkey);
+        if (rinfo & 0x00040004u) { const bool nA = (ia & CI_BASE_MASK) == 4, nB = (ib & CI_BASE_MASK) == 4; lane_rows<K, true, S8, TB, K3, NK>(s, P, sel, diag0, rf, nA, nB, acc, colkey, ofs); }
+        else          lane_rows<K, false, S8, TB, K3, NK>(s, P, sel, diag0, rf, false, false, acc, colkey, ofs);
         if constexpr (TB) {
             if (tb_a) {
                 if (TB_TILE > 1 && !RE) {
@@ -425,12 +463,12 @@
             s.best_hi = upB ? khi : s.best_hi; s.step_hi = upB ? t : s.step_hi;
             }
             if (rinfo & (CI_STORE_END * 0x00010001u)) {
-                if (vA && (ia & CI_STORE_END)) store_to_scratch<0, K>(s, P, s.probA, s.nodeA);
-                if (vB && (ib & CI_STORE_END)) store_to_scratch<1, K>(s, P, s.probB, s.nodeB);
+                if (vA && (ia & CI_STORE_END)) store_to_scratch<0, K>(s, P, s.probA, s.nodeA, floor2);
+                if (vB && (ib & CI_STORE_END)) store_to_scratch<1, K>(s, P, s.probB, s.nodeB, floor2);
             }
         }
     } else {
-        s.out_h = 0; s.out_f = 0;
+        s.out_h = floor2; s.out_f = floor2;
     }
     s.prev_rh = rh;
 }
@@ -438,10 +476,10 @@
 VGK_HD void steady_steps(uint32_t G, uint32_t shortest, uint32_t n_steps, uint32_t& from, uint32_t& to) {
     from = G - 1u < n_steps ? G - 1u : n_steps; to = shortest < n_steps ? shortest : n_steps; if (to < from) to = from;
 }
-template <int K, bool S8, bool TB = true, bool K3 = false, bool NK = false, bool AV = false>
+template <int K, bool S8, bool TB = true, bool K3 = false, bool NK = false, bool AV = false, int OFS = -1>
 VGK_HD void lane_step(Lane<K>& s, const GsswParams& P, uint32_t t, uint32_t rh, uint32_t rf, uint32_t rinfo, uint32_t* tb_a, uint32_t* tb_b) {
-    if (s.g == 0) { rh = 0; rf = 0; rinfo = fetch_info(s, P, t); }
-    lane_column<K, S8, TB, false, K3, NK, AV>(s, P, t, rh, rf, rinfo, tb_a, tb_b);
+    if (s.g == 0) { rh = rf = offset_rows<S8, TB, K3, OFS>(P) ? rep2(P.row_off) : 0u; rinfo = fetch_info(s, P, t); }
+    lane_column<K, S8, TB, false, K3, NK, AV, OFS>(s, P, t, rh, rf, rinfo, tb_a, tb_b);
 }
 
 template <int K>
@@ -934,7 +972,7 @@
 #if VGK_PB_LDS && defined(__HIPCC__)
     s.PBL = (typename Lane<K>::lds_u32*)(uintptr_t)0;
 #endif
-    lane_init(s, P, wd, lane);
+    lane_init<K, -1, 0>(s, P, wd, lane);
     const uint32_t g = s.g;
     uint32_t re[2] = {0, 0}, ce[2] = {0, 0}; TbBand bd[2]; bd[0].used = bd[1].used = false;
     const uint32_t prob[2] = {s.probA, s.probB};
diff --git a/vg_amd/csrc/pk16.hpp b/vg_amd/csrc/pk16.hpp
--- a/vg_amd/csrc/pk16.hpp
+++ b/vg_amd/csrc/pk16.hpp
@@ -1,5 +1,8 @@
 #pragma once
 #include <stdint.h>
+#if defined(VGK_PK_CHECK) && !defined(__HIPCC__)
+#include <atomic>
+#endif
 
 #if defined(__HIPCC__)
 #define VGK_HD __host__ __device__ __forceinline__
@@ -28,8 +31,12 @@
     uint32_t r; asm("v_bfi_b32 %0, %1, %2, %3" : "=v"(r) : "s"(MASK), "v"(a), "v"(b)); return r; }
 template <int N> static __device__ __forceinline__ uint32_t shl_or(uint32_t a, uint32_t c) {
     uint32_t r; asm("v_lshl_or_b32 %0, %1, %2, %3" : "=v"(r) : "v"(a), "n"(N), "v"(c)); return r; }
+template <int M> static __device__ __forceinline__ uint32_t pk_mul_imm_add_u(uint32_t a, uint32_t c) {
+    uint32_t r; asm("v_pk_mad_u16 %0, %1, %2, %3 op_sel_hi:[1,0,1]" : "=v"(r) : "v"(a), "n"(M), "s"(c)); return r; }
 static __device__ __forceinline__ uint32_t pk_max3_f16(uint32_t a, uint32_t b, uint32_t c) {
     uint32_t r; asm("v_pk_maximum3_f16 %0, %1, %2, %3" : "=v"(r) : "v"(a), "v"(b), "v"(c)); return r; }
+static __device__ __forceinline__ uint32_t pk_max3_f16_u(uint32_t a, uint32_t b, uint32_t c) {
+    uint32_t r; asm("v_pk_maximum3_f16 %0, %1, %2, %3" : "=v"(r) : "v"(a), "v"(b), "s"(c)); return r; }
 static __device__ __forceinline__ uint32_t pk_max_lo_into_hi(uint32_t a) {
     uint32_t r; asm("v_pk_max_u16 %0, %1, %1 op_sel:[0,0] op_sel_hi:[1,0]" : "=v"(r) : "v"(a)); return r; }
 static __device__ __forceinline__ uint32_t pk_max_bhi(uint32_t a, uint32_t b) {
@@ -52,7 +59,9 @@
 static inline uint32_t pk_min(uint32_t a, uint32_t b) { return pk_mk(pk_lo(a) < pk_lo(b) ? pk_lo(a) : pk_lo(b), pk_hi(a) < pk_hi(b) ? pk_hi(a) : pk_hi(b)); }
 static inline uint32_t pk_mad(uint32_t a, uint32_t b, uint32_t c) { return pk_mk(pk_lo(a) * pk_lo(b) + pk_lo(c), pk_hi(a) * pk_hi(b) + pk_hi(c)); }
 static inline uint32_t pk_max3_f16(uint32_t a, uint32_t b, uint32_t c) { return pk_max(pk_max(a, b), c); }
+static inline uint32_t pk_max3_f16_u(uint32_t a, uint32_t b, uint32_t c) { return pk_max3_f16(a, b, c); }
 template <int M> static inline uint32_t pk_mul_add_imm(uint32_t a, uint32_t c) { return pk_mad(a, (uint32_t)M * 0x00010001u, c); }
+template <int M> static inline uint32_t pk_mul_imm_add_u(uint32_t a, uint32_t c) { return pk_mad(a, (uint32_t)M * 0x00010001u, c); }
 template <int C> static inline uint32_t pk_mad_add_imm(uint32_t a, uint32_t b) { return pk_mad(a, b, (uint32_t)C * 0x00010001u); }
 static inline uint32_t byte_perm(uint32_t a, uint32_t b, uint32_t sel) {
     uint64_t src = ((uint64_t)a << 32) | b;
@@ -69,8 +78,15 @@
 }
 #endif
 
-VGK_HD uint32_t pk_add_nc(uint32_t a, uint32_t b) { return a + b; }
-VGK_HD uint32_t pk_sub_nb(uint32_t a, uint32_t b) { return a - b; }
+#if defined(VGK_PK_CHECK) && !defined(__HIPCC__)
+inline std::atomic<unsigned long long> pk_check_failures{0};
+inline void pk_check(bool ok) { if (!ok) pk_check_failures.fetch_add(1, std::memory_order_relaxed); }
+#define VGK_PK_EXPECT(X) pk_check(X)
+#else
+#define VGK_PK_EXPECT(X) ((void)0)
+#endif
+VGK_HD uint32_t pk_add_nc(uint32_t a, uint32_t b) { VGK_PK_EXPECT((a & 0xffffu) + (b & 0xffffu) < 0x10000u && (a >> 16) + (b >> 16) < 0x10000u); return a + b; }
+VGK_HD uint32_t pk_sub_nb(uint32_t a, uint32_t b) { VGK_PK_EXPECT((a & 0xffffu) >= (b & 0xffffu) && (a >> 16) >= (b >> 16)); return a - b; }
 
 VGK_HD uint32_t set_lo(uint32_t x, uint32_t v) { return (x & 0xffff0000u) | (v & 0xffffu); }
 VGK_HD uint32_t set_hi(uint32_t x, uint32_t v) { return (x & 0x0000ffffu) | (v << 16); }
diff --git a/vg_amd/csrc/vgk_api.cpp b/vg_amd/csrc/vgk_api.cpp
--- a/vg_amd/csrc/vgk_api.cpp
+++ b/vg_amd/csrc/vgk_api.cpp
@@ -440,12 +440,13 @@
     P.walk_passes = walk2 && !P.fused ? 2 : 1;
     if (P.walk_passes != 2 || P.tb_mode != TB_CODES) P.spec_fill = 0;
     set_refill_bound(P, ctx);
-    P.key3 = 0;
+    P.key3 = 0; P.row_off = 0;
     if (P.spec_fill) {
         uint32_t longest = 0; bool xdrop = false;
         for (uint32_t i = 0; i < n; ++i) { longest = std::max(longest, probs[i].L); xdrop = xdrop || (problems[i].flags & 15u) == (uint32_t)VGK_XDROP_PINNED; }
         P.key3 = gssw_key3_ok(S, ctx->has_qa, xdrop, longest, (uint32_t)std::max(0, ctx->max_score), (uint32_t)std::max(0, ctx->max_bonus)) && !std::getenv("VGAMD_NO_KEY3") ? 1u : 0u;
     }
+    P.row_off = P.key3 && !std::getenv("VGAMD_NO_OFFSET_ROWS") ? gssw_row_offset(S, P.go, P.ge, P.bias) : 0u;
     std::memcpy(P.matrix, ctx->sc.matrix, 25);
     b->ops_total = ops_total;
     if ((rc = ctx->be->sync_side())) return fail(rc);
@@ -721,6 +722,10 @@
     for (uint32_t i : list) if (i < b->n && probs[i].col0) ++out[3];
     return VGK_OK;
 } catch (const std::bad_alloc&) { return VGK_ENOMEM; } catch (...) { return VGK_EINVAL; }
+extern "C" uint32_t vgk_batch_row_offset(vgk_batch* b) { return b && b->P.spec_fill && b->P.key3 ? b->P.row_off : 0u; }
+#if defined(VGK_PK_CHECK)
+extern "C" uint64_t vgk_pk_check_failures(void) { return pk_check_failures.load(); }
+#endif
 int      vgk_batch_lane(vgk_batch* b) { return b ? b->lane : 0; }
 int      vgk_batch_speculated(vgk_batch* b) { if (!b) return 0; std::lock_guard<std::mutex> lk(b->ctx->mu); return b->ran && b->ran_spec ? 1 : 0; }
 int      vgk_set_speculation(vgk_ctx* ctx, int mode) {
diff --git a/vg_amd/csrc/window_api.cpp b/vg_amd/csrc/window_api.cpp
--- a/vg_amd/csrc/window_api.cpp
+++ b/vg_amd/csrc/window_api.cpp
@@ -293,12 +293,13 @@
     P.walk_passes = walk2 ? 2 : 1;
     if (P.walk_passes != 2 || P.tb_mode != TB_CODES) P.spec_fill = 0;
     set_refill_bound(P, ctx);
-    P.key3 = 0;
+    P.key3 = 0; P.row_off = 0;
     if (P.spec_fill) {
         uint32_t longest = 0; bool xdrop = false;
         for (uint32_t i = 0; i < n; ++i) { longest = std::max(longest, problems[i].read_len); xdrop = xdrop || (problems[i].flags & 15u) == (uint32_t)VGK_XDROP_PINNED; }
         P.key3 = gssw_key3_ok(S, ctx->has_qa, xdrop, longest, (uint32_t)std::max(0, ctx->max_score), (uint32_t)std::max(0, ctx->max_bonus)) && !std::getenv("VGAMD_NO_KEY3") ? 1u : 0u;
     }
+    P.row_off = P.key3 && !std::getenv("VGAMD_NO_OFFSET_ROWS") ? gssw_row_offset(S, P.go, P.ge, P.bias) : 0u;
     std::memcpy(P.matrix, ctx->sc.matrix, 25);
     b->ops_total = T.tot[WS_OPS]; b->wave_steps = T.wave_steps;
     lap("done");
```

New measurement: 75.92 million, median of 6. +5.7%, better.
